# r9y9/gantts

Hardware: AMD Instinct MI355X
Metric: acoustic frames/sec per G+D GAN step (B=32,T=512) (higher is better)
Workload: dtype f32; 1 GPU; cfg2: TTS acoustic MLP G 425-512x3-187 + conditioned MLP D 483-256x3-1, Adagrad, MGE+ADV loss, global B=32 T=512 (32 sequences per GPU, strong scaling), fp32, dropout 0.5 (Philox); global_batch=32, per_gpu_batch=32, parallelism=dp1

## Files before the change

gantts_amd/_lib.py:

```python
import ctypes as C
import os

import torch

_HERE = os.path.dirname(os.path.abspath(__file__))
LIB_PATH = os.environ.get("GT_HIP_LIB") or os.path.join(_HERE, "libgantts_hip.so")

GT_OK, GT_ERR_INVALID, GT_ERR_HIP, GT_ERR_STATE, GT_ERR_DIM = 0, 1, 2, 3, 4
ROLE_G, ROLE_D = 0, 1
OPT_LSTM_PERSISTENT, OPT_LSTM_FWD_UNITS, OPT_LSTM_XCD_LOCAL, OPT_MATMUL_BF16, OPT_SPLIT_FIRST_LAYER = 2, 3, 4, 5, 6
OPT_COMM_D_ONE_MSG, OPT_COMM_EARLY_G, OPT_COMM_FORCE = 10, 11, 13
OPT_LAUNCH_RIDERS, OPT_COMM_CLOSE_INLINE, OPT_POLL_RESULTS = 14, 15, 16
OPT_COMM_TV_IN_SUMS, OPT_COMM_IPC, OPT_FUSED_DSTACK = 17, 18, 19
OPT_SRU_D_BF16 = 20
OPT_GAN_OBJECTIVE = 21
GAN_OBJECTIVES = {"bce": 0, "ls": 1, "hinge": 2, "wgan": 3}
GAN_OBJECTIVE_THRESHOLD = {"bce": 0.5, "ls": 0.5, "hinge": 0.0, "wgan": 0.0}
IPC_HANDLE_BYTES, IPC_MAX_WORLD = 64, 8
PROFILE_SLOTS = 16
LSTM_PATH_SLOTS, LSTM_PATH_STEPS, LSTM_PATH_DECLINED = 34, 32, 33
GEMM_PATH_SLOTS = 588
GEMM_B16_PATH_SLOTS = 66
SRU_PATH_SLOTS = 13
HEAD_PATH_SLOTS = 15
SN_MAX_LAYERS, SN_PATH_SLOTS = 17, 5
GP_MAX_LAYERS, GP_PATH_SLOTS = 16, 8
GRAD_PENALTIES = {None: 0, "r1": 1, "wgan-gp": 2}
(FRAME_MASK_SUM, FRAME_MASK_TOTAL, FRAME_SQERR, FRAME_G_LOSSES, FRAME_STATIC_GRAD, FRAME_FINALIZE_G, FRAME_FINALIZE_G_RIDER, FRAME_FINALIZE_D,
 FRAME_SCALE_INV_TV, FRAME_HIGHWAY_FWD, FRAME_HIGHWAY_BWD, FRAME_SIGMOID_GRAD, FRAME_DROPOUT_APPLY, FRAME_BUILD_ADV, FRAME_BUILD_CAT2, FRAME_REPITCH,
 FRAME_DENSE_COPY, FRAME_PAD_ROWS, FRAME_TRANSPOSE) = range(19)
FRAME_SCALARS = 26
CAST_PLAIN_F32, CAST_PLAIN_BF16, CAST_SEQDROP, CAST_CAT, CAST_CATDROP, CAST_MULTI = 0, 1, 2, 3, 4, 5
CAST_MAX_JOBS = 8
GEMM_ROUTE_FORWARD, GEMM_ROUTE_FORWARD_SEG, GEMM_ROUTE_BACKWARD_DATA, GEMM_ROUTE_WEIGHT_GRAD, GEMM_ROUTE_WEIGHT_GRAD_SPLIT = 0, 1, 2, 3, 4
ARCH_MLP, ARCH_IN2OUT, ARCH_LSTM, ARCH_SRU, ARCH_IN2OUT_RNN = 0, 1, 2, 3, 4
OPT_ADAGRAD, OPT_ADAM = 0, 1
OPT_SGD, OPT_RMSPROP, OPT_ADADELTA, OPT_ADAMW, OPT_ADAMAX = 2, 3, 4, 5, 6
OPT_NADAM, OPT_RADAM, OPT_RPROP, OPT_ASGD = 7, 8, 9, 10
OPTF_NESTEROV, OPTF_CENTERED, OPTF_AMSGRAD, OPTF_BUFFER_LIVE = 1, 2, 4, 8
OPTF_DECOUPLED_WD = 32
MLPG_VAR_PATH_SLOTS = 3
MAX_STREAMS = 8
MLPG_R_FROM_WINDOWS = 1
MLPG_MAX_WINDOW_SPAN = 32
COMM_ID_BYTES = 128
SCALE_NONE, SCALE_MINMAX, SCALE_MEANVAR = 0, 1, 2
ASSEMBLE_MAX_WINDOWS, ASSEMBLE_MAX_TAPS = 4, 9
CORPUS_STATS_SLAB, CORPUS_STATS_FANIN = 256, 64
LEDGER_SLOTS = 32
LEDGER_HAS_D, LEDGER_HAS_G, LEDGER_HAS_DIST = 1, 2, 4
LEDGER_ACOUSTIC, LEDGER_DURATION, LEDGER_VC = 0, 1, 2
LEDGER_KEYS = ("generator", "mse", "mge", "loss_real_d", "loss_fake_d", "loss_adv", "discriminator", "real_correct", "fake_correct",
               "mcd", "bap_mcd", "f0_rmse", "vuv_err", "dur_rmse", "d_updates", "g_updates")


class StreamConfig(C.Structure):
    _fields_ = [("n_streams", C.c_int32),
                ("stream_sizes", C.c_int32 * MAX_STREAMS),
                ("has_dynamic_features", C.c_int32 * MAX_STREAMS),
                ("num_windows", C.c_int32),
                ("adversarial_streams", C.c_int32 * MAX_STREAMS),
                ("mask_nth_mgc_for_adv_loss", C.c_int32),
                ("discriminator_linguistic_condition", C.c_int32),
                ("cond_dim", C.c_int32)]


class ModelDesc(C.Structure):
    _fields_ = [("arch", C.c_int32), ("in_dim", C.c_int32), ("out_dim", C.c_int32),
                ("num_hidden", C.c_int32), ("hidden_dim", C.c_int32), ("static_dim", C.c_int32),
                ("dropout", C.c_float), ("last_sigmoid", C.c_int32),
                ("bidirectional", C.c_int32), ("use_relu", C.c_int32),
                ("rnn_dropout", C.c_float), ("reserved_", C.c_int32),
                ("params", C.c_void_p), ("grads", C.c_void_p), ("n_params", C.c_int64)]


class OptimDesc(C.Structure):
    _fields_ = [("kind", C.c_int32), ("lr", C.c_float), ("weight_decay", C.c_float), ("eps", C.c_float),
                ("lr_decay", C.c_float), ("beta1", C.c_float), ("beta2", C.c_float),
                ("max_grad_norm", C.c_float), ("step", C.c_int64),
                ("state0", C.c_void_p), ("state1", C.c_void_p)]


class OptimDescEx(C.Structure):
    _fields_ = ([("kind", C.c_int32), ("flags", C.c_uint32)]
                + [(n, C.c_double) for n in ("lr", "weight_decay", "eps", "lr_decay", "beta1", "beta2", "momentum", "dampening", "alpha")]
                + [("max_grad_norm", C.c_float), ("reserved_", C.c_int32), ("step", C.c_int64),
                   ("state0", C.c_void_p), ("state1", C.c_void_p), ("state2", C.c_void_p)])


class OptimDescEx2(OptimDescEx):
    _fields_ = [(n, C.c_double) for n in ("momentum_decay", "etaminus", "etaplus", "step_size_min", "step_size_max", "lambd", "t0",
                                          "host_state0", "host_state1")]


class DResult(C.Structure):
    _fields_ = [("loss_d", C.c_float), ("loss_fake_d", C.c_float), ("loss_real_d", C.c_float),
                ("real_correct_count", C.c_float), ("fake_correct_count", C.c_float), ("grad_norm", C.c_float)]


class GResult(C.Structure):
    _fields_ = [("loss_mse", C.c_float), ("loss_mge", C.c_float), ("loss_adv", C.c_float),
                ("loss_g", C.c_float), ("grad_norm", C.c_float)]


class GemmCase(C.Structure):
    _fields_ = ([(n, C.c_int32) for n in ("route", "prec", "rows", "in_dim", "out_dim", "act", "drop")] + [("p", C.c_float)]
                + [("key0", C.c_uint32), ("key1", C.c_uint32)]
# ... 97 lines not shown

class GpCase(C.Structure):
    _fields_ = ([(n, C.c_int32) for n in ("kind", "L", "H", "cd", "Da", "ld_g")] + [("rows", C.c_int64), ("weight", C.c_float), ("inv_tv", C.c_float)]
                + [(n, C.c_void_p * GP_MAX_LAYERS) for n in ("W", "dW", "Hact", "a", "c")] + [("drop", DropSite * GP_MAX_LAYERS)]
                + [(n, C.c_void_p) for n in ("w_last", "dw_last", "mask", "g", "g_copy", "phi", "nrm", "sums", "rec")])


class CastJob(C.Structure):
    _fields_ = ([(n, C.c_void_p) for n in ("in_", "out", "outT")] + [("rows", C.c_int64), ("ldt", C.c_int64)]
                + [(n, C.c_int32) for n in ("ldi", "cols", "ldo", "pad_")])


class CastCase(C.Structure):
    _fields_ = ([(n, C.c_int32) for n in ("kind", "cols", "ldi", "ldo", "colsum_accumulate", "T", "cd", "ldf", "n_jobs", "pad_")]
                + [(n, C.c_int64) for n in ("rows", "ldt", "N", "row_off")]
                + [(n, C.c_void_p) for n in ("in_", "out", "outT", "colsum", "mul", "x", "fa", "fb", "idx")]
                + [("jobs", CastJob * CAST_MAX_JOBS)])


_P, _I, _F, _L = C.c_void_p, C.c_int, C.c_float, C.c_int64

class DistortionSums(C.Structure):
    _fields_ = [(n, C.c_double) for n in
                ("s_mcd", "s_bap", "s_f0", "n_voiced", "n_vuv_err", "s_mse", "n_frames")]


SIGNATURES = {
    "gt_last_error": (C.c_char_p, []),
    "gt_version": (C.c_char_p, []),
    "gt_engine_create": (_I, [C.POINTER(StreamConfig), C.POINTER(_P)]),
    "gt_engine_destroy": (None, [_P]),
    "gt_bind_model": (_I, [_P, _I, C.POINTER(ModelDesc)]),
    "gt_bind_optimizer": (_I, [_P, _I, C.POINTER(OptimDesc)]),
    "gt_bind_optimizer_ex": (_I, [_P, _I, C.POINTER(OptimDescEx)]),
    "gt_op_optim_step": (_I, [C.POINTER(OptimDescEx), _P, _P, _L, _P, C.POINTER(_F), _P]),
    "gt_set_training": (_I, [_P, _I, _I]),
    "gt_set_lr": (_I, [_P, _I, _F]),
    "gt_get_optimizer_step": (_I, [_P, _I, C.POINTER(_L)]),
    "gt_get_optimizer_scalars": (_I, [_P, _I, C.POINTER(C.c_double)]),
    "gt_op_optim_scalars": (_I, [C.POINTER(OptimDescEx), _L, C.POINTER(C.c_double)]),
    "gt_set_seed": (_I, [_P, C.c_uint64]),
    "gt_set_dropout_mask": (_I, [_P, _I, _I, _I, _P]),
    "gt_op_philox_mask": (_I, [_P, _I, _I, _I, _L, _F, _L, _I, _P, _P]),
    "gt_set_lengths": (_I, [_P, C.POINTER(_L), _I, _P]),
    "gt_invalidate_mlpg_cache": (_I, [_P]),
    "gt_set_mlpg_windows": (_I, [_P, _I, C.POINTER(C.c_int32), C.POINTER(C.c_int32), C.POINTER(C.c_double)]),
    "gt_zero_grad": (_I, [_P, _I]),
    "gt_apply_generator": (_I, [_P, _P, _P, _I, _I, _P, _P, _P]),
    "gt_update_discriminator": (_I, [_P, _P, _P, _P, _P, _I, _I, _I, _F, C.POINTER(DResult), _P]),
    "gt_update_generator": (_I, [_P, _P, _P, _P, _P, _P, _F, _P, _I, _I, _I, _F, _F, _F, C.POINTER(GResult), _P]),
    "gt_set_loss_normalizer": (_I, [_P, _F]),
    "gt_set_loss_normalizer_device": (_I, [_P, _P]),
    "gt_set_option": (_I, [_P, _I, _I]),
    "gt_set_weight_clip": (_I, [_P, _I, _F]),
    "gt_set_param_ema": (_I, [_P, _I, _P, _L, C.c_double]),
    "gt_set_param_ema_count": (_I, [_P, _I, _L]),
    "gt_get_param_ema_count": (_I, [_P, _I, C.POINTER(_L)]),
    "gt_op_optim_step_ema": (_I, [C.POINTER(OptimDescEx), _P, _P, _L, _P, C.POINTER(_F), _P, _L, C.c_double, _P]),
    "gt_set_spectral_norm": (_I, [_P, _I, _P, _P, _L, _L]),
    "gt_op_spectral_norm": (_I, [C.POINTER(SnCase), _P]),
    "gt_op_sn_project": (_I, [C.POINTER(SnCase), _P]),
    "gt_sn_path_counts": (_I, [C.POINTER(_L), _I]),
    "gt_set_grad_penalty": (_I, [_P, _I, _I, _F]),
    "gt_set_gp_epsilon": (_I, [_P, _P]),
    "gt_grad_penalty_result": (_I, [_P, C.POINTER(C.c_double), C.POINTER(C.c_double), C.POINTER(_L), _I]),
    "gt_grad_penalty_peek": (_I, [_P, _P, _P, _P]),
    "gt_op_grad_penalty": (_I, [C.POINTER(GpCase), _P]),
    "gt_gp_path_counts": (_I, [C.POINTER(_L), _I]),
    "gt_set_x_pitch": (_I, [_P, _I, _I]),
    "gt_set_tuning": (_I, [C.c_char_p, _I]),
    "gt_check_faults": (_I, [_P, _P]),
    "gt_lstm_path_counts": (_I, [_P, C.POINTER(_L), _I]),
    "gt_gemm_path_counts": (_I, [C.POINTER(_L), _I]),
    "gt_op_gemm_f32": (_I, [C.POINTER(GemmCase), _P]),
    "gt_gemm_b16_path_counts": (_I, [C.POINTER(_L), _I]),
    "gt_op_gemm_b16": (_I, [C.POINTER(GemmB16Case), _P]),
    "gt_op_cast_image": (_I, [C.POINTER(CastCase), _P]),
    "gt_sru_path_counts": (_I, [C.POINTER(_L), _I]),
    "gt_op_sru_scan": (_I, [C.POINTER(SruScanCase), _P]),
    "gt_op_sru_dx_adv_finish": (_I, [_P, _L, _I, _I, _P, _I, _P, _I, _P]),
    "gt_op_sru_input_mask": (_I, [_P, _I, _I, _F, C.c_uint32, C.c_uint32, _P, _I, _I, _P]),
    "gt_op_sru_input_dropout": (_I, [_P, _I, _P, _I, _I, _I, _I, _P, _P]),
    "gt_head_path_counts": (_I, [C.POINTER(_L), _I]),
    "gt_op_d_head": (_I, [C.POINTER(DHeadCase), _P]),
    "gt_op_dstack": (_I, [C.POINTER(DStackCase), _P]),
    "gt_op_frame": (_I, [C.POINTER(FrameCase), _P]),
    "gt_op_mlpg": (_I, [C.POINTER(MlpgCase), _P]),
    "gt_op_mlpg_band": (_I, [_P, _P, _I, C.POINTER(_F), _L, C.POINTER(C.c_int32), _P]),
    "gt_op_mlpg_var": (_I, [C.POINTER(MlpgVarCase), _P]),
    "gt_mlpg_var_path_counts": (_I, [C.POINTER(_L), _I]),
    "gt_op_assemble_batch": (_I, [C.POINTER(AssembleCase), _P]),
    "gt_op_assemble_shard": (_I, [C.POINTER(AssembleCase), C.POINTER(AssembleShard), _P]),
    "gt_corpus_stats_workspace_bytes": (_L, [_L, C.c_int32]),
    "gt_op_corpus_stats": (_I, [C.POINTER(CorpusStatsCase), _P]),
    "gt_clear_faults": (_I, [_P, _P]),
    "gt_comm_unique_id": (_I, [_P]),
    "gt_comm_init": (_I, [_P, _I, _I, _P]),
    "gt_comm_destroy": (_I, [_P]),
    "gt_comm_info": (_I, [_P, C.POINTER(_I), C.POINTER(_I)]),
    "gt_comm_trace": (_I, [_P, _I]),
    "gt_comm_trace_read": (_I, [_P, C.POINTER(C.c_double), _I, C.POINTER(_I)]),
    "gt_set_shard": (_I, [_P, _I, _I]),
    "gt_comm_ipc_export": (_I, [_P, _P]),
    "gt_comm_ipc_attach": (_I, [_P, _I, _I, _P]),
    "gt_comm_ipc_messages": (_I, [_P, C.POINTER(C.c_longlong)]),
    "gt_update_discriminator_begin": (_I, [_P, _P, _P, _P, _P, _I, _I, _I, _F, _P]),
    "gt_update_discriminator_end": (_I, [_P, _I, C.POINTER(DResult), _P]),
    "gt_update_generator_begin": (_I, [_P, _P, _P, _P, _P, _P, _F, _P, _I, _I, _I, _F, _F, _F, _P]),
    "gt_update_generator_end": (_I, [_P, _I, _F, _F, _F, C.POINTER(GResult), _P]),
    "gt_update_discriminator_result": (_I, [_P, C.POINTER(DResult)]),
    "gt_update_generator_result": (_I, [_P, C.POINTER(GResult)]),
    "gt_scalar_buffer": (_I, [_P, C.POINTER(_P), C.POINTER(_I)]),
    "gt_model_forward": (_I, [_P, _I, _P, _P, _I, _I, _P, _P, _P]),
    "gt_flush_generator_grads": (_I, [_P, _P]),
    "gt_op_sequence_mask": (_I, [_P, _I, _I, _P, _P]),
    "gt_op_masked_mse": (_I, [_P, _P, _P, _I, _I, _I, C.POINTER(_F), _P, _P]),
    "gt_compute_distortions": (_I, [_P, _P, _I, _P, _P, _I, C.POINTER(_I), C.POINTER(_I), _I, C.POINTER(_L), _I, _I,
                                    C.POINTER(DistortionSums), _P]),
    "gt_ledger_configure": (_I, [_P, _I, _I, C.POINTER(_I), C.POINTER(_I), _I, _P, _P, _I, C.c_double]),
    "gt_ledger_reset": (_I, [_P, _P]),
    "gt_ledger_add": (_I, [_P, _I, _P, _P, _P, _I, _I, _P]),
    "gt_ledger_read": (_I, [_P, C.POINTER(C.c_double), _P]),
    "gt_ledger_buffers": (_I, [_P, C.POINTER(_P), C.POINTER(_P)]),
    "gt_op_epoch_ledger": (_I, [_P, _P, _P, _I, _I, _I, C.c_double, _P]),
    "gt_host_wait_count": (_I, [_P, C.POINTER(C.c_longlong)]),
    "gt_op_gather_cols": (_I, [_P, _I, _P, _I, _P, _I, _I, _L, _P]),
    "gt_op_pad_sequences": (_I, [_P, _I, _P, _P, _I, _I, _P, _I, _P]),
    "gt_op_mlpg_forward": (_I, [_P, _P, _P, _I, _I, _P, _P]),
    "gt_op_mlpg_backward": (_I, [_P, _P, _P, _I, _I, _P, _P]),
    "gt_op_linear_forward": (_I, [_P, _I, _P, _P, _P, _I, _L, _I, _I, _I, _P, _F, _P]),
    "gt_op_linear_bf16": (_I, [_P, _P, _P, _L, _I, _I, _I, _P, _F, _P, _P, _P, _I, _P, _F, _P, _P, _P, _P, _P, _P]),
    "gt_profile_enable": (_I, [_I]),
    "gt_profile_read": (_I, [C.POINTER(C.c_double), C.POINTER(C.c_double), C.POINTER(_L)]),
    "gt_profile_bytes": (_I, [C.POINTER(C.c_double)]),
    "gt_op_linear_backward": (_I, [_P, _I, _P, _I, _P, _L, _I, _I, _P, _I, _P, _I, _P, _F, _P, _P, _P]),
}


def _build_if_missing():
    import fcntl
    import shutil
    import subprocess
    if os.path.isfile(LIB_PATH):
        return
    if shutil.which("hipcc") is None and not os.path.isfile("/opt/rocm/bin/hipcc"):
        return
    with open(os.path.join(_HERE, ".build.lock"), "w") as lock:
        fcntl.flock(lock, fcntl.LOCK_EX)
        try:
            if not os.path.isfile(LIB_PATH):
                subprocess.call(["make", "-j8", "-C", os.path.join(_HERE, "csrc")], stdout=subprocess.DEVNULL)
        finally:
            fcntl.flock(lock, fcntl.LOCK_UN)


def _load():
    _build_if_missing()
    if not os.path.isfile(LIB_PATH):
        raise ImportError(
            "gantts_amd: %s not found -- the HIP engine is the product and has no fallback. "
            "Build it: make -C %s" % (LIB_PATH, os.path.join(_HERE, "csrc")))
    lib = C.CDLL(LIB_PATH)
    for name, (res, args) in SIGNATURES.items():
        fn = getattr(lib, name)
        fn.restype, fn.argtypes = res, args
    return lib
# ... 30 lines not shown
```

gantts_amd/csrc/d_tail_args.hip.h:

```cpp
#pragma once
#include "dstack_f32.hip.h"

namespace gt {

struct HeadCall {
  int mode;
  long rows, n_real;
  const float* mask; long n_mask;
  float eps;
  bool want_grad;
  bool want_w;
  StepResults* early_res;
  int* defer_scalars;
  const double* tv_dev;
  unsigned ticket;
  bool unit_tv;
  int objective;
};

struct HeadSums {
  StepScalars* sc;
  HeadPartials* hp; long hp_cap;
  float* dw_partial; long dw_cap;
  float* dW; float* db;
  int accumulate;
  unsigned* ticket_dev;
};

struct HeadArgs {
  HeadCall c;
  HeadSums o;
  const void* H; int K;
  int ldh;
  int h_ld;
  bool has_act;
  DropoutSpec spec;
  const float* w; const float* bias;
  float* Dout;
  float* dH; int lddh;
  __bf16* dHb; int lddhb;
  __bf16* dHbT; long lddhbt;
};

struct DStackCall {
  HeadCall c;
  HeadSums o;
  int hidden_dim;
  DStackArgs a;
};

inline int d_head_blocks(long rows) { const long n = (rows + 31) / 32; return (int)(n < 1024 ? n : 1024); }

}
```

gantts_amd/csrc/eng_core.hip:

```cpp
#include "engine_internal.hip.h"

using namespace gt;
static thread_local char g_err[512] = "";
int fail(int code, const char* fmt, ...) {
  va_list ap;
  va_start(ap, fmt);
  vsnprintf(g_err, sizeof(g_err), fmt, ap);
  va_end(ap);
  return code;
}
extern "C" const char* gt_last_error(void) { return g_err; }
extern "C" const char* gt_version(void) { return "gantts_hip 0.1 (gfx950, f32 MFMA)"; }

int ensure_dyn_lds(const void* kernel, size_t bytes) {
  static std::mutex mu;
  static std::map<std::pair<const void*, int>, size_t> done;
  int dev = 0;
  HIPCHK(hipGetDevice(&dev));
  std::lock_guard<std::mutex> lk(mu);
  size_t& cur = done[std::make_pair(kernel, dev)];
  if (bytes > cur) {
    HIPCHK(hipFuncSetAttribute(kernel, hipFuncAttributeMaxDynamicSharedMemorySize, (int)bytes));
    cur = bytes;
  }
// ... 325 lines not shown
extern "C" int gt_set_training(gt_engine* e, int role, int training) {
  if (!e || role < 0 || role > 1) return fail(GT_ERR_INVALID, "bad argument");
  e->net[role].training = training != 0;
  return GT_OK;
}
extern "C" int gt_set_lr(gt_engine* e, int role, float lr) {
  if (!e || role < 0 || role > 1 || !e->net[role].has_opt) return fail(GT_ERR_INVALID, "no optimizer bound");
  e->net[role].od.lr = lr;
  return GT_OK;
}
extern "C" int gt_get_optimizer_step(gt_engine* e, int role, int64_t* step) {
  if (!e || role < 0 || role > 1 || !step) return fail(GT_ERR_INVALID, "bad argument");
  *step = e->net[role].step;
  return GT_OK;
}
extern "C" int gt_get_optimizer_scalars(gt_engine* e, int role, double out[2]) {
  if (!e || role < 0 || role > 1 || !out) return fail(GT_ERR_INVALID, "bad argument");
  Net& n = e->net[role];
  if (!n.has_opt) return fail(GT_ERR_INVALID, "no optimizer bound");
  optim_host_scalars(n.od, n.step, &n.hs_cache, out);
  return GT_OK;
}
extern "C" int gt_set_seed(gt_engine* e, uint64_t seed) {
  if (!e) return fail(GT_ERR_INVALID, "null engine");
  e->seed = seed;
  e->step_counter = 0;
  e->dx_pitched.forget(); e->gx_pitched.forget(); e->cx_dense.forget();
  return GT_OK;
}
extern "C" int gt_set_dropout_mask(gt_engine* e, int role, int pass, int layer, const float* mask) {
  if (!e || role < 0 || role > 1 || pass < 0 || pass > (role == GT_ROLE_D ? 3 : 2) || layer < 0 || layer > 15) return fail(GT_ERR_INVALID, "bad argument");
  e->net[role].inj[pass][layer] = mask;
  return GT_OK;
}
extern "C" int gt_set_option(gt_engine* e, int option, int value) {
  if (!e) return fail(GT_ERR_INVALID, "null engine");
  switch (option) {
    case GT_OPT_LSTM_PERSISTENT: e->lstm_persistent = value != 0; return GT_OK;
    case GT_OPT_LSTM_FWD_UNITS: e->lstm_fwd_upc = value; return GT_OK;
    case GT_OPT_LSTM_XCD_LOCAL: e->lstm_xcd_local = value != 0; return GT_OK;
    case GT_OPT_SPLIT_FIRST_LAYER:
      if (e->opt_split_first != (value != 0)) invalidate_d_images(e);
      e->opt_split_first = value != 0;
      return GT_OK;
    case GT_OPT_COMM_D_ONE_MSG: e->opt_comm_d_one_msg = value != 0; return GT_OK;
    case GT_OPT_COMM_EARLY_G: e->opt_comm_early_g = value != 0; return GT_OK;
    case GT_OPT_COMM_FORCE: e->opt_comm_force = value != 0; return GT_OK;
    case GT_OPT_COMM_CLOSE_INLINE: e->opt_comm_close_inline = value != 0; return GT_OK;
    case GT_OPT_COMM_IPC: e->opt_comm_ipc = value != 0; return GT_OK;
    case GT_OPT_FUSED_DSTACK: e->opt_fused_dstack = value < 0 ? 0 : value > 2 ? 2 : value; return GT_OK;
    case GT_OPT_COMM_TV_IN_SUMS: e->opt_comm_tv_in_sums = value != 0; return GT_OK;
    case GT_OPT_POLL_RESULTS: e->opt_poll_results = value != 0; return GT_OK;
    case GT_OPT_LAUNCH_RIDERS: e->opt_launch_riders = value != 0; return GT_OK;
    case GT_OPT_MATMUL_BF16:
      if (e->matmul_bf16 != (value != 0)) {
        invalidate_d_images(e);
        e->g_pass_valid = false; e->leak.drop(); e->cx_dense.forget(); e->results.forget_begin();
      }
      e->matmul_bf16 = value != 0;
      return GT_OK;
    case GT_OPT_SRU_D_BF16:
      if (value != 0 && value != 1) return fail(GT_ERR_INVALID, "GT_OPT_SRU_D_BF16 takes 0 or 1, not %d", value);
      if (e->sru_d_bf16 != (value != 0)) { invalidate_d_images(e); e->leak.drop(); e->results.forget_begin(); }
      e->sru_d_bf16 = value != 0;
      return GT_OK;
    case GT_OPT_GAN_OBJECTIVE:
      if (value < 0 || value >= GAN_OBJ_COUNT) return fail(GT_ERR_INVALID, "GT_OPT_GAN_OBJECTIVE takes 0 (bce), 1 (ls), 2 (hinge) or 3 (wgan), not %d", value);
      if (e->net[GT_ROLE_D].bound) CHK(gan_objective_fits(value, e->net[GT_ROLE_D].d.last_sigmoid != 0));
      if (e->gan_objective != value) { e->leak.drop(); e->results.forget_begin(); }
      e->gan_objective = value;
      return GT_OK;
  }
  return fail(GT_ERR_INVALID, "unknown option %d", option);
}
GtTuning& gt_tuning() {
  static GtTuning t = [] {
    GtTuning v;
    auto geti = [](const char* n, int d) { const char* s = getenv(n); return s && s[0] ? atoi(s) : d; };
    v.gemm_pair = geti("GT_GEMM_PAIR", v.gemm_pair); v.pair_order = geti("GT_PAIR_ORDER", v.pair_order);
    { const char* s = getenv("GT_GEMM_TILES"); v.gemm_tiles_big = s && !strcmp(s, "big") ? 1 : 0; }
    v.gemm_unaligned = geti("GT_GEMM_UNALIGNED", v.gemm_unaligned); v.tn_wgs = geti("GT_TN_WGS", v.tn_wgs); v.tn_split_wgs = geti("GT_TN_SPLIT_WGS", v.tn_split_wgs); v.split_fused = geti("GT_SPLIT_FUSED", v.split_fused);
    v.b16_tiles = geti("GT_B16_TILES", v.b16_tiles); v.b16_wg_tile = geti("GT_B16_WG_TILE", v.b16_wg_tile); v.b16_dma = geti("GT_B16_DMA", v.b16_dma);
    v.mlpg_fpl = geti("GT_MLPG_FPL", v.mlpg_fpl); v.mlpg_tt = geti("GT_MLPG_TT", v.mlpg_tt); v.sru_coop = geti("GT_SRU_COOP", v.sru_coop); v.sru_cs_waves = geti("GT_SRU_CS_WAVES", v.sru_cs_waves); v.leak_rider = geti("GT_LEAK_RIDER", v.leak_rider);
    v.head_vec = geti("GT_HEAD_VEC", v.head_vec);
    v.lstm_bt = geti("GT_LSTM_BT", v.lstm_bt);
    if (v.lstm_bt != 8 && v.lstm_bt != 16) v.lstm_bt = 0;
    return v;
  }();
  return t;
}
extern "C" int gt_set_tuning(const char* name, int value) {
  if (!name) return fail(GT_ERR_INVALID, "null name");
  GtTuning& t = gt_tuning();
  struct { const char* n; int* p; } tab[] = {
      {"gemm_pair", &t.gemm_pair}, {"pair_order", &t.pair_order}, {"gemm_tiles_big", &t.gemm_tiles_big}, {"gemm_unaligned", &t.gemm_unaligned},
      {"tn_wgs", &t.tn_wgs}, {"tn_split_wgs", &t.tn_split_wgs}, {"split_fused", &t.split_fused}, {"b16_tiles", &t.b16_tiles},
      {"b16_wg_tile", &t.b16_wg_tile}, {"b16_dma", &t.b16_dma}, {"mlpg_fpl", &t.mlpg_fpl}, {"mlpg_tt", &t.mlpg_tt}, {"sru_coop", &t.sru_coop}, {"sru_cs_waves", &t.sru_cs_waves}, {"leak_rider", &t.leak_rider}, {"head_vec", &t.head_vec}};
  if (!strcmp(name, "lstm_bt")) {
    if (value != 0 && value != 8 && value != 16) return fail(GT_ERR_INVALID, "lstm_bt must be 0 (by shape), 8 or 16, not %d", value);
    t.lstm_bt = value;
    return GT_OK;
  }
  if (!strcmp(name, "sru_lw")) { t.sru_coop = value >= 2; return GT_OK; }
  for (auto& e : tab) if (!strcmp(e.n, name)) { *e.p = value; return GT_OK; }
  return fail(GT_ERR_INVALID, "unknown tuning knob '%s'", name);
}
extern "C" int gt_set_x_pitch(gt_engine* e, int ld_generator_input, int ld_condition) {
  if (!e || ld_generator_input < 0 || ld_condition < 0) return fail(GT_ERR_INVALID, "bad argument");
  e->ld_gx = ld_generator_input; e->ld_cx = ld_condition;
  return GT_OK;
}
extern "C" int gt_set_loss_normalizer(gt_engine* e, float tv) {
  if (!e) return fail(GT_ERR_INVALID, "null engine");
  e->norm.set_override(tv);
  return GT_OK;
}
extern "C" int gt_set_loss_normalizer_device(gt_engine* e, const double* tv_dev) {
  if (!e) return fail(GT_ERR_INVALID, "null engine");
  e->norm.set_total_dev(tv_dev);
  return GT_OK;
}
extern "C" int gt_set_lengths(gt_engine* e, const int64_t* lengths_host, int B, void* stream) {
  if (!e || !lengths_host || B < 1) return fail(GT_ERR_INVALID, "bad argument");
  hipStream_t s = (hipStream_t)stream;
  e->h_lengths.resize(B);
  for (int b = 0; b < B; ++b) {
    if (lengths_host[b] < 0 || lengths_host[b] > 0x3fffffff) return fail(GT_ERR_INVALID, "length out of range");
    e->h_lengths[b] = (int)lengths_host[b];
  }
  if (2 * B > e->len_cap) {
    HIPCHK(hipStreamSynchronize(s));
    const int cap = std::max(64, 2 * B + B);
    for (int i = 0; i < gt_engine::LEN_RING; ++i) {
      if (e->len_ev[i]) HIPCHK(hipEventSynchronize(e->len_ev[i]));
      if (e->len_host[i]) { HIPCHK(hipHostFree(e->len_host[i])); e->len_host[i] = nullptr; }
      HIPCHK(hipHostMalloc((void**)&e->len_host[i], (size_t)cap * sizeof(int)));
      if (!e->len_ev[i]) HIPCHK(hipEventCreateWithFlags(&e->len_ev[i], hipEventDisableTiming));
    }
    e->len_cap = cap;
  }
  const int slot = (e->len_slot + 1) % gt_engine::LEN_RING;
  HIPCHK(hipEventSynchronize(e->len_ev[slot]));
  memcpy(e->len_host[slot], e->h_lengths.data(), (size_t)B * sizeof(int));
  memcpy(e->len_host[slot] + B, e->h_lengths.data(), (size_t)B * sizeof(int));
  CHK(e->len_dev[slot].ensure((size_t)e->len_cap * sizeof(int)));
  HIPCHK(hipMemcpyAsync(e->len_dev[slot].p, e->len_host[slot], (size_t)2 * B * sizeof(int), hipMemcpyHostToDevice, s));
  HIPCHK(hipEventRecord(e->len_ev[slot], s));
  e->len_slot = slot;
  return GT_OK;
}

extern "C" int gt_zero_grad(gt_engine* e, int role) {
  if (!e || role < 0 || role > 1) return fail(GT_ERR_INVALID, "bad argument");
  e->net[role].grads_dirty = false;
  e->ws[role].sdefer.reset(false);
  e->norm.forget();
  if (role == GT_ROLE_G) e->leak.drop();
  return GT_OK;
}
extern "C" int gt_scalar_buffer(gt_engine* e, double** dev_ptr, int* n) {
  if (!e || !dev_ptr || !n) return fail(GT_ERR_INVALID, "bad argument");
  *dev_ptr = &e->sc()->s_real;
  *n = 7;
  return GT_OK;
}

DropoutSpec philox_site_spec(gt_engine* e, int role, int pass, int layer, uint64_t step, float p, long half_rows) {
  DropoutSpec d = no_drop();
  d.p = p;
  d.scale = 1.f / (1.f - p);
  d.mode = DROP_PHILOX;
  const double th = (double)p * 65536.0 + 0.5;
  d.thresh = th >= 65535.0 ? 65535u : (uint32_t)th;
  const uint64_t site = step * 64ULL + (uint64_t)(role * 32 + pass * 16 + layer);
  uint32_t rk = 0;
  if (e->dp_world > 1) {
    const int T = e->chk_T, B = e->chk_B;
    const long groups = ((long)B * T / 16) * e->dp_world * 2;
    if (T > 0 && T % 16 == 0 && groups < (1L << 21) && (half_rows == 0 || half_rows == (long)B * T)) {
      d.dp_t16 = (uint32_t)(T / 16);
// ... 90 lines not shown
```

gantts_amd/csrc/eng_gemm_f32.hip:

```cpp
#include "engine_internal.hip.h"
#include <atomic>

using namespace gt;
int launch_gemm_nt(const GemmArgs& g, int bm, int bn, int prec, hipStream_t s);
int launch_gemm_nn(const GemmArgs& g, int bm, int bn, int prec, hipStream_t s);
int launch_gemm_tn(const GemmArgs& g, int bm, int bn, int nslab, int prec, hipStream_t s);
int launch_gemm_pair(const GemmArgs& nn_in, const GemmArgs& tn_in, int nslab, int prec, hipStream_t s);
int launch_gemm_tn_pair(const GemmArgs& g1_in, const GemmArgs& g2_in, int nslab1, int nslab2, int prec, hipStream_t s, const GemmArgs* rider, bool* rode);
int gemm_cu_count() {
  static std::map<int, int> cus;
  int dev = 0;
  if (hipGetDevice(&dev) != hipSuccess) return 256;
  auto it = cus.find(dev);
  if (it != cus.end()) return it->second;
  hipDeviceProp_t prop;
  const int n = hipGetDeviceProperties(&prop, dev) == hipSuccess ? prop.multiProcessorCount : 256;
  cus[dev] = n;
  return n;
}

static std::atomic<int64_t> g_gemm_paths[GT_GEMM_PATH_SLOTS];
void gemm_path_count(int slot) { g_gemm_paths[slot].fetch_add(1, std::memory_order_relaxed); }
extern "C" int gt_gemm_path_counts(int64_t* counts, int reset) {
  for (int i = 0; i < GT_GEMM_PATH_SLOTS; ++i) {
    const int64_t v = reset ? g_gemm_paths[i].exchange(0, std::memory_order_relaxed) : g_gemm_paths[i].load(std::memory_order_relaxed);
    if (counts) counts[i] = v;
  }
  return GT_OK;
}

static int pick_bn(int N) { return (cdiv(N, 64) * 64 < cdiv(N, 128) * 128) ? 64 : 128; }

static int gemm_tile_mode() { return gt_tuning().gemm_tiles_big; }
static bool gemm_unaligned_ok() { return gt_tuning().gemm_unaligned != 0; }
bool gemm_vec_ok(const float* p, int ld, bool k_contiguous) {
  if (k_contiguous && gemm_unaligned_ok()) return true;
  return (ld % 4 == 0) && (((uintptr_t)p) % 16 == 0);
}
bool gemm_wide_store_ok(int kind, const GemmArgs& g) {
  if (kind == GEMM_TN) return false;
  if (gemm_unaligned_ok()) return true;
  return (g.ldc % 4 == 0) && (((uintptr_t)g.C) % 16 == 0) &&
         (kind != GEMM_NN || g.act == ACT_NONE || ((g.ldh % 4 == 0) && (((uintptr_t)g.H) % 16 == 0)));
}
bool gemm_small_tiles_ok() { return gemm_tile_mode() == 0; }


int launch_gemm(int kind, const GemmArgs& g, int prec, hipStream_t s) {
  if (g.M <= 0 || g.N <= 0 || g.K <= 0) return fail(GT_ERR_INVALID, "empty GEMM");
  if (kind != GEMM_NT && kind != GEMM_NN) return fail(GT_ERR_INVALID, "launch_gemm: forward and backward-data products only");
  const bool nt = kind == GEMM_NT;
  const bool vec = gemm_vec_ok(g.A, g.lda, true) && gemm_vec_ok(g.B, g.ldb, nt);
  if (vec && g.M > 64 && gemm_small_tiles_ok()) return nt ? launch_gemm_nt(g, 64, 64, prec, s) : launch_gemm_nn(g, 64, 64, prec, s);
  const int bn = pick_bn(g.N);
  int bm = 128;
  if (g.M > 64) {
    const long t128 = (long)cdiv(g.M, 128) * cdiv(g.N, bn), t64 = (long)cdiv(g.M, 64) * cdiv(g.N, bn);
    const double c128 = (double)cdiv(t128, 512), c64 = 0.55 * (double)cdiv(t64, bn == 64 ? 1024 : 768);
    if (c64 < c128) bm = 64;
  }
  return nt ? launch_gemm_nt(g, bm, bn, prec, s) : launch_gemm_nn(g, bm, bn, prec, s);
}
static int launch_gemm_slabs(const GemmArgs& g, int tile_m, int nslab, int prec, hipStream_t s) {
  if (g.M <= 0 || g.N <= 0 || g.K <= 0) return fail(GT_ERR_INVALID, "empty GEMM");
  return tile_m == 64 ? launch_gemm_tn(g, 64, 64, nslab, prec, s) : launch_gemm_tn(g, 128, pick_bn(g.N), nslab, prec, s);
}

DropoutSpec no_drop() {
  DropoutSpec d;
  memset(&d, 0, sizeof(d));
  d.mode = DROP_NONE;
  d.scale = 1.f;
  return d;
}
static GemmArgs gemm_args(const float* A, int lda, const float* B, int ldb, float* C, int ldc, long M, int N, int K) {
  GemmArgs g;
  memset(&g, 0, sizeof(g));
  g.A = A; g.lda = lda; g.B = B; g.ldb = ldb; g.C = C; g.ldc = ldc; g.M = (int)M; g.N = N; g.K = K;
  g.drop = no_drop();
  return g;
}
int plain_product(int kind, const float* A, int lda, const float* B, int ldb, float* C, int ldc, long M, int N, int K, bool accumulate, int prec,
                  hipStream_t s) {
  GemmArgs g = gemm_args(A, lda, B, ldb, C, ldc, M, N, K);
  g.accumulate = accumulate ? 1 : 0;
  return launch_gemm(kind, g, prec, s);
}

int linear_forward(const float* X, int ldx, const float* W, int ldw, const float* b, float* Y, int ldy, long rows, int in, int out, int act,
                   const DropoutSpec& drop, int prec, hipStream_t s, const float* addm, int ld_addm, long addm_wrap, bool accumulate) {
  GemmArgs g = gemm_args(X, ldx, W, ldw, Y, ldy, rows, out, in);
  g.bias = b; g.act = act; g.drop = drop; g.accumulate = accumulate ? 1 : 0;
  if (addm) { g.addm = addm; g.ld_addm = ld_addm; g.addm_wrap = (int)addm_wrap; }
  return launch_gemm(GEMM_NT, g, prec, s);
}
int linear_forward_seg(const float* x, int ldx, long wrap, int cd, const float* adv, int ld_adv, long rows, const float* W, int ldw, int in,
                       const float* b, float* Y, int ldy, int out, int act, const DropoutSpec& drop, int prec, hipStream_t s) {
  GemmArgs g = gemm_args(x, ldx, W, ldw, Y, ldy, wrap, out, cd);
  g.bias = b; g.act = act; g.drop = drop;
  g.A_seg = adv; g.lda_seg = ld_adv; g.B_seg = W + cd; g.K_seg = in - cd;
  g.dual_rows = rows == 2 * wrap ? (int)wrap : 0;
  return launch_gemm(GEMM_NT, g, prec, s);
}
GemmArgs backward_data_args(const float* dZ, int lddz, const float* W, int ldw, int col0, float* dX, int lddx,
                                   long rows, int out, int ncols, int act_prev, const float* H, int ldh, const DropoutSpec& drop) {
  GemmArgs g = gemm_args(dZ, lddz, W + col0, ldw, dX, lddx, rows, ncols, out);
  g.act = act_prev; g.H = H; g.ldh = ldh; g.drop = drop;
  return g;
}
int linear_backward_data(const float* dZ, int lddz, const float* W, int ldw, int col0, float* dX, int lddx,
                                long rows, int out, int ncols, int act_prev, const float* H, int ldh,
                                const DropoutSpec& drop, int prec, hipStream_t s) {
  return launch_gemm(GEMM_NN, backward_data_args(dZ, lddz, W, ldw, col0, dX, lddx, rows, out, ncols, act_prev, H, ldh, drop), prec, s);
}
static bool gemm_pair_enabled() { return gt_tuning().gemm_pair != 0; }
static bool gemm_pair_ok(const GemmArgs& nn) {
  return gemm_pair_enabled() && gemm_small_tiles_ok() && nn.M > 64 && gemm_vec_ok(nn.A, nn.lda, true) && gemm_vec_ok(nn.B, nn.ldb);
}


int slab_defer_flush(SlabDefer& d, hipStream_t s) {
  if (d.jobs.n > 0) {
    gemm_path_count(GEMM_PATH_REDUCE_MULTI);
    hipLaunchKernelGGL(slab_reduce_multi_kernel, dim3(d.blocks), dim3(256), 0, s, d.jobs);
    LAUNCH_CHECK();
  }
  d.jobs.n = 0; d.blocks = 0; d.used = 0;
  return GT_OK;
}
int slab_place(SlabDefer* defer, Scratch& slabs, int nslab, int out, int in, const float* dW, bool accumulate, hipStream_t s, SlabSet* set) {
  const long stride = (long)out * in;
  const size_t need = (((size_t)nslab * stride + (size_t)nslab * out) * sizeof(float) + 255) & ~(size_t)255;
  const bool can4 = stride % 4 == 0 && ((uintptr_t)dW) % 16 == 0;
  float* base = nullptr;
  if (defer && defer->active && accumulate) { CHK(slab_defer_flush(*defer, s)); defer = nullptr; }
  if (defer && defer->active && can4) {
    if (defer->jobs.n == SLAB_MAX_JOBS || defer->used + need > defer->pool.bytes) {
      CHK(slab_defer_flush(*defer, s));
      if (need > defer->pool.bytes) CHK(defer->pool.ensure(std::max(need * 4, (size_t)64 << 20)));
    }
    base = (float*)((char*)defer->pool.p + defer->used);
    defer->used += need;
  } else {
    defer = nullptr;
    CHK(slabs.ensure(need));
    base = slabs.as<float>();
  }
  *set = SlabSet{base, base + (size_t)nslab * stride, stride, need, nslab, out, can4, defer};
  return GT_OK;
}
int slab_combine(const SlabSet& t, float* dW, float* db, bool accumulate, hipStream_t s) {
  const int acc = accumulate ? 1 : 0;
  if (t.can4) {
    const int main_blocks = cdiv(t.stride / 4, 256), bias_blocks = db ? cdiv(t.out, 256) : 0;
    if (SlabDefer* d = t.defer) {
      SlabJob& J = d->jobs.j[d->jobs.n++];
      J.slabs = t.base; J.slab_stride = t.stride; J.n4 = t.stride / 4; J.out = dW; J.bslabs = t.bias; J.bout = db;
      J.nslab = t.nslab; J.accumulate = acc; J.nb = t.out; J.main_blocks = main_blocks; J.block0 = d->blocks; J.pad_ = 0;
      d->blocks += main_blocks + bias_blocks;
      return GT_OK;
    }
    gemm_path_count(GEMM_PATH_REDUCE4);
    hipLaunchKernelGGL(slab_reduce4_kernel, dim3(main_blocks + bias_blocks), dim3(256), 0, s, t.base, t.stride, t.nslab, t.stride / 4, dW, acc,
                       (const float*)t.bias, t.out, db, main_blocks);
    LAUNCH_CHECK();
    return GT_OK;
  }
  gemm_path_count(GEMM_PATH_REDUCE);
  hipLaunchKernelGGL(slab_reduce_kernel, dim3(cdiv(t.stride, 256)), dim3(256), 0, s, t.base, t.stride, t.nslab, t.stride, dW, acc);
  LAUNCH_CHECK();
  if (db) {
    gemm_path_count(GEMM_PATH_REDUCE_SMALL);
    hipLaunchKernelGGL(slab_reduce_small_kernel, dim3(cdiv(t.out, 64)), dim3(1024), 0, s, t.bias, (long)t.out, t.nslab, t.out, db, acc);
    LAUNCH_CHECK();
  }
  return GT_OK;
}
int linear_backward_weight(const float* dZ, int lddz, const float* X, int ldx, long rows, int out, int in,
                                  float* dW, float* db, bool accumulate, Scratch& slabs, Scratch& colp, int prec, hipStream_t s,
                                  SlabDefer* defer, const GemmArgs* ride_along, bool* rode) {
  if (rode) *rode = false;
  if (dW) {
    const bool t64 = gemm_vec_ok(dZ, lddz) && gemm_vec_ok(X, ldx) && gemm_small_tiles_ok();
    const int bn = t64 ? 64 : pick_bn(in);
    const int tiles = cdiv(out, t64 ? 64 : 128) * cdiv(in, bn);
    const int slab_wgs = gt_tuning().tn_wgs;
    int nslab = std::max(1, slab_wgs / tiles);
    const int max_slab = (int)((rows + 255) / 256);
    if (nslab > max_slab) nslab = max_slab;
    if (nslab < 1) nslab = 1;
    int k_chunk = cdiv(cdiv(rows, nslab), GEMM_BK) * GEMM_BK;
    nslab = cdiv(rows, k_chunk);
    SlabSet set;
    CHK(slab_place(defer, slabs, nslab, out, in, dW, accumulate, s, &set));
    GemmArgs g = gemm_args(dZ, lddz, X, ldx, set.base, in, out, in, (int)rows);
    g.k_chunk = k_chunk; g.slab_stride = set.stride;
    g.colsum_slab = db ? set.bias : nullptr;
    if (t64 && ride_along && rode && gemm_pair_ok(*ride_along)) {
      CHK(launch_gemm_pair(*ride_along, g, nslab, prec, s));
      *rode = true;
    } else {
      CHK(launch_gemm_slabs(g, t64 ? 64 : 128, nslab, prec, s));
    }
    return slab_combine(set, dW, db, accumulate, s);
  }
  if (db) {
    const int rows_per_blk = 128;
    const int nblk = cdiv(rows, rows_per_blk);
    CHK(colp.ensure((size_t)nblk * out * sizeof(float)));
    gemm_path_count(GEMM_PATH_COLSUM_PARTIAL);
    hipLaunchKernelGGL(colsum_partial_kernel, dim3(nblk, cdiv(out, 64)), dim3(256), 0, s, dZ, lddz, rows, out, rows_per_blk,
                       colp.as<float>());
    LAUNCH_CHECK();
    gemm_path_count(GEMM_PATH_COLSUM_FINALIZE);
    hipLaunchKernelGGL(colsum_finalize_kernel, dim3(cdiv(out, 256)), dim3(256), 0, s, colp.as<float>(), nblk, out, db,
                       accumulate ? 1 : 0);
    LAUNCH_CHECK();
  }
  return GT_OK;
}


int linear_backward_weight_split(const float* dZ, int lddz, long rows, long wrap, const float* xp, int ldxp, int cd,
                                 const float* adv, int ld_adv, int Da, int out, float* dW, float* db, bool accumulate,
                                 Scratch& slabs, int prec, hipStream_t s, SlabDefer* defer, const GemmArgs* rider, bool* rode) {
  if (rode) *rode = false;
  if (rows != wrap && rows != 2 * wrap) return fail(GT_ERR_INVALID, "split weight gradient: rows must be one or two halves");
  if (!gemm_vec_ok(dZ, lddz) || !gemm_vec_ok(xp, ldxp) || !gemm_vec_ok(adv, ld_adv) || prec != PREC_F32)
    return fail(GT_ERR_INVALID, "split weight gradient: operands must be 16-byte loadable (float32 products)");
  const int in = cd + Da;
  const int tiles = cdiv(out, 64) * (cdiv(cd, 64) + cdiv(Da, 64));
  int nslab = std::max(1, gt_tuning().tn_split_wgs / tiles);
  nslab = std::min<long>(nslab, std::max<long>(1, wrap / 256));
  const int kc1 = cdiv(cdiv(wrap, nslab), GEMM_BK) * GEMM_BK;
  const int ns1 = cdiv(wrap, kc1);
  const int kc2 = cdiv(cdiv(rows, ns1), GEMM_BK) * GEMM_BK;
  const int ns2 = cdiv(rows, kc2);
  SlabSet set;
  CHK(slab_place(defer, slabs, ns1, out, in, dW, accumulate, s, &set));
  if (ns2 < ns1)
    HIPCHK(hipMemsetAsync(set.base, 0, set.bytes, s));
  GemmArgs g1 = gemm_args(dZ, lddz, xp, ldxp, set.base, in, out, cd, (int)wrap);
  g1.A2 = rows == 2 * wrap ? dZ + wrap * (long)lddz : nullptr;
  g1.k_chunk = kc1; g1.slab_stride = set.stride;
  GemmArgs g2 = g1;
  g2.A2 = nullptr; g2.B = adv; g2.ldb = ld_adv; g2.C = set.base + cd; g2.N = Da; g2.K = (int)rows; g2.k_chunk = kc2;
  g2.colsum_slab = db ? set.bias : nullptr;
  if (g1.A2) {
    CHK(launch_gemm_tn_pair(g1, g2, ns1, ns2, prec, s, rider, rode));
  } else {
    CHK(launch_gemm_slabs(g1, 64, ns1, prec, s));
    CHK(launch_gemm_slabs(g2, 64, ns2, prec, s));
  }
  return slab_combine(set, dW, db, accumulate, s);
}
```

gantts_amd/csrc/eng_gemm_f32_pair.hip:

```cpp
#include "gemm_f32_launch.hip.h"

int launch_gemm_pair(const GemmArgs& nn_in, const GemmArgs& tn_in, int nslab, int prec, hipStream_t s) {
  GemmArgs nn = nn_in, tn = tn_in;
  nn.wide_store = gemm_wide_store_ok(GEMM_NN, nn) ? 1 : 0;
  tn.wide_store = 0;
  nn.n_tiles_m = cdiv(nn.M, 64); nn.n_tiles_n = cdiv(nn.N, 64);
  tn.n_tiles_m = cdiv(tn.M, 64); tn.n_tiles_n = cdiv(tn.N, 64);
  const int n1 = nn.n_tiles_m * nn.n_tiles_n, n2 = tn.n_tiles_m * tn.n_tiles_n * nslab;
  const bool bf16 = prec == PREC_BF16;
  const size_t lds = bf16 ? std::max(gemm_lds_bytes<GEMM_NN, 64, 64, PREC_BF16>(), gemm_lds_bytes<GEMM_TN, 64, 64, PREC_BF16>())
                          : std::max(gemm_lds_bytes<GEMM_NN, 64, 64>(), gemm_lds_bytes<GEMM_TN, 64, 64>());
  const int am = bf16 ? GEMM_A_RUNTIME : (nn.act == ACT_NONE ? GEMM_A_NONE : ((nn.act == ACT_LEAKY_DROPOUT && nn.drop.mode == DROP_PHILOX) ? GEMM_A_LEAKY_PHILOX : GEMM_A_RUNTIME));
  const void* kern = bf16 ? (const void*)gemm_pair_kernel<PREC_BF16> : (am == GEMM_A_NONE ? (const void*)gemm_pair_kernel<PREC_F32, GEMM_A_NONE> :
                     (am == GEMM_A_LEAKY_PHILOX ? (const void*)gemm_pair_kernel<PREC_F32, GEMM_A_LEAKY_PHILOX> : (const void*)gemm_pair_kernel<PREC_F32>));
  CHK(ensure_dyn_lds(kern, lds));
  GemmProfiler::Rec rec;
  if (g_prof.wants(5)) {
    rec.kind = 5; rec.bn = 64; rec.am = -1; rec.flops = 2.0 * nn.M * nn.N * nn.K + 2.0 * tn.M * tn.N * tn.K;
    rec.bytes = gemm_algorithmic_bytes(GEMM_NN, nn) + gemm_algorithmic_bytes(GEMM_TN, tn);
    rec.e0 = g_prof.get(); rec.e1 = g_prof.get();
    HIPCHK(hipEventRecord(rec.e0, s));
  }
  const int tn_first = gt_tuning().pair_order;
  const int grid = n1 + n2;
  gemm_path_count(GEMM_PATH_PAIR + (bf16 ? 3 : am == GEMM_A_NONE ? 0 : am == GEMM_A_LEAKY_PHILOX ? 1 : 2));
  if (bf16) hipLaunchKernelGGL(gemm_pair_kernel<PREC_BF16>, dim3(grid), dim3(GEMM_THREADS), lds, s, nn, tn, n1, tn_first);
  else if (am == GEMM_A_NONE) hipLaunchKernelGGL((gemm_pair_kernel<PREC_F32, GEMM_A_NONE>), dim3(grid), dim3(GEMM_THREADS), lds, s, nn, tn, n1, tn_first);
  else if (am == GEMM_A_LEAKY_PHILOX) hipLaunchKernelGGL((gemm_pair_kernel<PREC_F32, GEMM_A_LEAKY_PHILOX>), dim3(grid), dim3(GEMM_THREADS), lds, s, nn, tn, n1, tn_first);
  else      hipLaunchKernelGGL(gemm_pair_kernel<PREC_F32>, dim3(grid), dim3(GEMM_THREADS), lds, s, nn, tn, n1, tn_first);
  LAUNCH_CHECK();
  if (g_prof.wants(5)) { HIPCHK(hipEventRecord(rec.e1, s)); g_prof.recs.push_back(rec); }
  return GT_OK;
}

int launch_gemm_tn_pair(const GemmArgs& g1_in, const GemmArgs& g2_in, int nslab1, int nslab2, int prec, hipStream_t s, const GemmArgs* rider, bool* rode) {
  GemmArgs g1 = g1_in, g2 = g2_in, g3;
  memset(&g3, 0, sizeof(g3));
  int n3 = 0;
  if (rode) *rode = false;
  if (rider && rider->act == ACT_NONE && !rider->accumulate && rider->M > 0 && gemm_vec_ok(rider->A, rider->lda, true) && prec == PREC_F32 &&
      gemm_small_tiles_ok()) {
    g3 = *rider;
    g3.wide_store = gemm_wide_store_ok(GEMM_NN, g3) ? 1 : 0;
    g3.n_tiles_m = cdiv(g3.M, 64); g3.n_tiles_n = cdiv(g3.N, 64);
    n3 = g3.n_tiles_m * g3.n_tiles_n;
    if (rode) *rode = true;
  }
  g1.wide_store = g2.wide_store = 0;
  g1.n_tiles_m = cdiv(g1.M, 64); g1.n_tiles_n = cdiv(g1.N, 64);
  g2.n_tiles_m = cdiv(g2.M, 64); g2.n_tiles_n = cdiv(g2.N, 64);
  const int n1 = g1.n_tiles_m * g1.n_tiles_n * nslab1, n2 = g2.n_tiles_m * g2.n_tiles_n * nslab2;
  const size_t lds = std::max(gemm_lds_bytes<GEMM_TN, 64, 64>(), gemm_lds_bytes<GEMM_NN, 64, 64>());
  CHK(ensure_dyn_lds((const void*)gemm_tn_pair_kernel<PREC_F32>, lds));
  GemmProfiler::Rec rec;
  if (g_prof.wants(6)) {
    rec.kind = 6; rec.bn = 64; rec.am = -1; rec.flops = 2.0 * g1.M * g1.N * g1.K + 2.0 * g2.M * g2.N * g2.K + (n3 ? 2.0 * g3.M * g3.N * g3.K : 0.0);
    rec.bytes = gemm_algorithmic_bytes(GEMM_TN, g1) + 4.0 * (double)g1.M * g1.K + gemm_algorithmic_bytes(GEMM_TN, g2) + (n3 ? gemm_algorithmic_bytes(GEMM_NN, g3) : 0.0);
    rec.e0 = g_prof.get(); rec.e1 = g_prof.get();
    HIPCHK(hipEventRecord(rec.e0, s));
  }
  gemm_path_count(GEMM_PATH_TN_PAIR + (n3 > 0 ? 1 : 0));
  hipLaunchKernelGGL(gemm_tn_pair_kernel<PREC_F32>, dim3(n1 + n2 + n3), dim3(GEMM_THREADS), lds, s, g1, g2, n1, g3, n3);
  LAUNCH_CHECK();
  if (g_prof.wants(6)) { HIPCHK(hipEventRecord(rec.e1, s)); g_prof.recs.push_back(rec); }
  return GT_OK;
}
```

gantts_amd/csrc/eng_step.hip:

```cpp
#include "engine_internal.hip.h"
#include "d_tail_args.hip.h"
#include "d_tail_launch.hip.h"
#include <atomic>

using namespace gt;
static int stage_injected(gt_engine* e, int role, int layer, const int* passes, int npass, long rows_each, int width,
                          const float** out, hipStream_t s) {
  Net& n = e->net[role];
  *out = nullptr;
  if (!n.training || n.d.dropout <= 0.f) return GT_OK;
  bool any = false, all = true;
  for (int i = 0; i < npass; ++i) { any |= n.inj[passes[i]][layer] != nullptr; all &= n.inj[passes[i]][layer] != nullptr; }
  if (!any) return GT_OK;
  if (!all) return fail(GT_ERR_INVALID, "injected dropout masks must be given for every pass of a step or for none");
  if (npass == 1) { *out = n.inj[passes[0]][layer]; return GT_OK; }
  const size_t per_layer = (size_t)npass * rows_each * width * sizeof(float);
  CHK(e->dmask.ensure(per_layer * n.d.num_hidden));
  float* base = (float*)((char*)e->dmask.p + per_layer * layer);
  for (int i = 0; i < npass; ++i)
    HIPCHK(hipMemcpyAsync(base + (size_t)i * rows_each * width, n.inj[passes[i]][layer], (size_t)rows_each * width * sizeof(float),
                          hipMemcpyDeviceToDevice, s));
  *out = base;
  return GT_OK;
}

struct FirstSplit {
  const float* x; int ldx; int cd;
  const float* xp; int ldxp;
  const float* adv; int ld_adv;
  long wrap;
};
static int step_copy(gt_engine* e, StepCopy& M, const float* p, int ld, int cols, long rows, int ldo, bool dense, const float** out, hipStream_t s) {
  if (!M.holds(p, ld, cols, rows, e->step_counter)) {
    CHK(M.buf.ensure((size_t)rows * ldo * sizeof(float)));
    if (dense) launch_copy_cols(p, ld, 0, M.buf.as<float>(), ldo, 0, rows, cols, s);
    else launch_repitch(p, ld, cols, rows, M.buf.as<float>(), ldo, s);
    LAUNCH_CHECK();
    M.built(p, ld, cols, rows, e->step_counter);
  }
  *out = M.buf.as<float>();
  return GT_OK;
}
static int pitched_rows(gt_engine* e, StepCopy& M, const float* p, int ld, int cols, long rows, const float** out, int* ldo, hipStream_t s) {
  if (gemm_vec_ok(p, ld)) { *out = p; *ldo = ld; return GT_OK; }
  *ldo = (cols + 3) & ~3;
  return step_copy(e, M, p, ld, cols, rows, *ldo, false, out, s);
}

static int stack_forward(gt_engine* e, int role, const float* in, int ld_in, long rows, const int* passes, int npass, long rows_each, std::vector<DropoutSpec>& specs, hipStream_t s,
                         const FirstSplit* fs = nullptr, int max_layers = 1 << 30 ) {
  Net& n = e->net[role];
  std::vector<Scratch>& acts = e->ws[role].act;
  const int prec = product_prec(e, role);
  specs.resize(n.hidden.size());
  const float* cur = in;
  int ld = ld_in;
  for (size_t l = 0; l < n.hidden.size(); ++l) {
    const Lin& L = n.hidden[l];
    CHK(acts[l].ensure((size_t)rows * L.out * sizeof(float)));
    const float* inj = nullptr;
    CHK(stage_injected(e, role, (int)l, passes, npass, rows_each, L.out, &inj, s));
    specs[l] = drop_spec(e, role, passes[0], (int)l, inj, L.out, npass == 2 ? rows_each : 0);
    if ((int)l >= max_layers) continue;
    if (l == 0 && fs && specs[l].mode == DROP_PHILOX && gt_tuning().split_fused && gemm_vec_ok(fs->x, fs->ldx, true) &&
        gemm_vec_ok(L.W, L.in, true) && gemm_vec_ok(fs->adv, fs->ld_adv, true) && fs->wrap > 64 && gemm_small_tiles_ok() &&
        prec == PREC_F32 && (rows == fs->wrap || rows == 2 * fs->wrap)) {
      CHK(linear_forward_seg(fs->x, fs->ldx, fs->wrap, fs->cd, fs->adv, fs->ld_adv, rows, L.W, L.in, L.in, L.b, acts[l].as<float>(), L.out, L.out,
                             ACT_LEAKY_DROPOUT, specs[l], prec, s));
      cur = acts[l].as<float>();
      ld = L.out;
      continue;
    }
    if (l == 0 && fs) {
      const int Da = L.in - fs->cd;
      CHK(e->d_pre.ensure((size_t)fs->wrap * L.out * sizeof(float)));
      CHK(linear_forward(fs->x, fs->ldx, L.W, L.in, L.b, e->d_pre.as<float>(), L.out, fs->wrap, fs->cd, L.out, ACT_NONE, no_drop(), prec, s));
      CHK(linear_forward(fs->adv, fs->ld_adv, L.W + fs->cd, L.in, nullptr, acts[l].as<float>(), L.out, rows, Da, L.out, ACT_LEAKY_DROPOUT, specs[l],
                         prec, s, e->d_pre.as<float>(), L.out, fs->wrap));
      cur = acts[l].as<float>();
      ld = L.out;
      continue;
    }
    const float* W = L.W;
    int ldw = L.in;
    if (l == 0 && (L.in & 3) && gemm_vec_ok(cur, ld) && !gemm_vec_ok(L.W, L.in, true) && prec == PREC_F32) {
      ldw = (L.in + 3) & ~3;
      CHK(e->ws[role].w0pad.ensure((size_t)L.out * ldw * sizeof(float)));
      launch_pad_rows(L.W, L.in, L.out, e->ws[role].w0pad.as<float>(), ldw, s);
      LAUNCH_CHECK();
      W = e->ws[role].w0pad.as<float>();
    }
    CHK(linear_forward(cur, ld, W, ldw, L.b, acts[l].as<float>(), L.out, rows, L.in, L.out, ACT_LEAKY_DROPOUT, specs[l], prec, s));
    cur = acts[l].as<float>();
    ld = L.out;
  }
  return GT_OK;
}


static int stack_backward(gt_engine* e, int role, const float* in, int ld_in, long rows, const std::vector<DropoutSpec>& specs, float* cur, float* other, bool want_w,
                          float* dX, int lddx, int col0, int ncols, long row0, long nrows, hipStream_t s, const FirstSplit* fs = nullptr) {
  Net& n = e->net[role];
  std::vector<Scratch>& acts = e->ws[role].act;
  const int L = (int)n.hidden.size(), prec = product_prec(e, role);
  for (int l = L - 1; l >= 0; --l) {
    const Lin& Lr = n.hidden[l];
    const float* Xin = l > 0 ? acts[l - 1].as<float>() : in;
    const int ldx = l > 0 ? n.hidden[l - 1].out : ld_in;
    bool rode = false;
    GemmArgs nn;
    if (l > 0) nn = backward_data_args(cur, Lr.out, Lr.W, Lr.in, 0, other, Lr.in, rows, Lr.out, Lr.in, ACT_LEAKY_DROPOUT,
                                       acts[l - 1].as<float>(), Lr.in, specs[l - 1]);
    if (want_w && l == 0 && fs) {
      GemmArgs leak;
      if (dX) leak = backward_data_args(cur + row0 * Lr.out, Lr.out, Lr.W, Lr.in, col0, dX, lddx, nrows, Lr.out, ncols, ACT_NONE, nullptr, 0, no_drop());
      CHK(linear_backward_weight_split(cur, Lr.out, rows, fs->wrap, fs->xp, fs->ldxp, fs->cd, fs->adv, fs->ld_adv, Lr.in - fs->cd, Lr.out,
                                       Lr.dW, Lr.db, n.grads_dirty, e->slabs, prec, s, &e->ws[role].sdefer, dX && gt_tuning().leak_rider ? &leak : nullptr, &rode));
      CHK(comm_grads_ready(e, role, Lr.dW, (long)Lr.out * Lr.in + Lr.out, s));
    } else if (want_w) {
      CHK(linear_backward_weight(cur, Lr.out, Xin, ldx, rows, Lr.out, Lr.in, Lr.dW, Lr.db, n.grads_dirty, e->slabs, e->colp, prec, s, &e->ws[role].sdefer,
                                 l > 0 ? &nn : nullptr, &rode));
      CHK(comm_grads_ready(e, role, Lr.dW, (long)Lr.out * Lr.in + Lr.out, s));
      if (l == 1 && (role == GT_ROLE_G || !e->opt_comm_d_one_msg)) CHK(comm_flush(e, role, s));
    }
    if (l > 0) {
      if (!rode) CHK(launch_gemm(GEMM_NN, nn, prec, s));
      std::swap(cur, other);
    } else if (dX && !rode) {
      CHK(linear_backward_data(cur + row0 * Lr.out, Lr.out, Lr.W, Lr.in, col0, dX, lddx, nrows, Lr.out, ncols, ACT_NONE, nullptr, 0,
                               no_drop(), prec, s));
    }
  }
  return GT_OK;
}

static bool use_b16(const gt_engine* e, int role) {
  const Net& n = e->net[role];
  if (!e->matmul_bf16 || !n.bound || n.d.arch != GT_ARCH_MLP || (n.d.hidden_dim & 7)) return false;
  return true;
}
static int refresh_shadows(gt_engine* e, int role, bool with_last, hipStream_t s) {
  Net& n = e->net[role];
  auto& sh = e->ws[role].wsh;
  sh.resize(n.hidden.size() + 1);
  CastJobs jobs;
  jobs.n = 0; jobs.pad_ = 0;
  int blocks = 0;
  auto flush = [&]() -> int {
    CHK(cast_transpose_multi(jobs, blocks, s));
    jobs.n = 0; blocks = 0;
    return GT_OK;
  };
  for (size_t l = 0; l <= n.hidden.size(); ++l) {
    if (l == n.hidden.size() && !with_last) break;
    const Lin& L = l < n.hidden.size() ? n.hidden[l] : n.last;
    LinShadow& w = sh[l];
    CHK(w.ensure(L.out, L.in));
    if (jobs.n == CAST_MAX_JOBS) CHK(flush());
    CHK(cast_jobs_add(jobs, blocks, L.W, L.in, L.out, L.in, w.r(), w.ldw, w.t(), w.ldwt));
  }
  return flush();
}
static int stack_forward_b16(gt_engine* e, int role, const __bf16* in_b, int ld_in, long rows, const int* passes, int npass, long rows_each,
                             std::vector<DropoutSpec>& specs, bool want_t, hipStream_t s) {
  Net& n = e->net[role];
  std::vector<B16Img>& acts = e->ws[role].actb;
  const std::vector<LinShadow>& wsh = e->ws[role].wsh;
  specs.resize(n.hidden.size());
  acts.resize(n.hidden.size());
  const __bf16* cur = in_b;
  int ld = ld_in;
  for (size_t l = 0; l < n.hidden.size(); ++l) {
    const Lin& L = n.hidden[l];
    CHK(acts[l].ensure(rows, L.out, want_t));
    const float* inj = nullptr;
    CHK(stage_injected(e, role, (int)l, passes, npass, rows_each, L.out, &inj, s));
    specs[l] = drop_spec(e, role, passes[0], (int)l, inj, L.out, npass == 2 ? rows_each : 0);
    CHK(b16_forward(cur, ld, rows, wsh[l].r(), wsh[l].ldw, L.out, L.in, L.b, ACT_LEAKY_DROPOUT, specs[l], B16Dst(acts[l], want_t), s));
    cur = acts[l].r();
    ld = acts[l].ld;
  }
  return GT_OK;
}
static int stack_backward_b16(gt_engine* e, int role, const __bf16* in_t, long ld_int, long rows, const std::vector<DropoutSpec>& specs, int cur, bool want_w,
                              float* dX, int lddx, int col0, int ncols, long row0, long nrows, hipStream_t s) {
  Net& n = e->net[role];
  std::vector<B16Img>& acts = e->ws[role].actb;
  const std::vector<LinShadow>& wsh = e->ws[role].wsh;
  for (int l = (int)n.hidden.size() - 1; l >= 0; --l) {
    const Lin& Lr = n.hidden[l];
    B16Img& dz = e->dz_b[cur];
    if (want_w) {
      const __bf16* XT = l > 0 ? acts[l - 1].t() : in_t;
      const long ldxt = l > 0 ? acts[l - 1].ldt : ld_int;
      CHK(weight_grad_b16(dz.t(), dz.ldt, XT, ldxt, rows, Lr.out, Lr.in, Lr.dW, Lr.db, n.grads_dirty, e->slabs, s, &e->ws[role].sdefer));
      CHK(comm_grads_ready(e, role, Lr.dW, (long)Lr.out * Lr.in + Lr.out, s));
      if (l == 1 && (role == GT_ROLE_G || !e->opt_comm_d_one_msg)) CHK(comm_flush(e, role, s));
    }
    if (l > 0) {
      B16Img& nx = e->dz_b[cur ^ 1];
      CHK(nx.ensure(rows, Lr.in, want_w));
      CHK(b16_backward_data(dz.r(), dz.ld, rows, wsh[l].t(), wsh[l].ldwt, Lr.in, Lr.out, ACT_LEAKY_DROPOUT, &acts[l - 1], specs[l - 1],
                            B16Dst(nx, want_w), s));
      cur ^= 1;
// ... 104 lines not shown
    }
    CHK(out_layer_forward(e, GT_ROLE_G, mlp_top(e, GT_ROLE_G, b16), N, y_hat, s));
  }
  if (is_i2o(G.d.arch)) {
    if (!R) return fail(GT_ERR_INVALID, "In2OutHighwayNet needs the MLPG matrix R (models.py:54)");
    const int sd = G.d.static_dim;
    const MlpgBand* band;
    CHK(ensure_band(e, R, T, s, &band));
    if (stash) e->g_band = band;
    CHK(e->tx.ensure((size_t)N * sd * sizeof(float)));
    CHK(e->gx.ensure((size_t)N * sd * sizeof(float)));
    CHK(linear_forward(x, G.d.in_dim, G.gate.W, sd, G.gate.b, e->tx.as<float>(), sd, N, sd, sd, ACT_SIGMOID, no_drop(), product_prec(e, GT_ROLE_G), s));
    CHK(mlpg_forward(e, gsrc, G.d.out_dim, e->d_scol_i2o, e->d_sstride_i2o, sd, e->gx.as<float>(), sd, B, T, *band, s));
    launch_highway_forward(x, G.d.in_dim, e->tx.as<float>(), sd, e->gx.as<float>(), sd, y_hat_static, sd, N, sd, s);
    LAUNCH_CHECK();
  } else {
    if (G.d.out_dim != e->Dout_cfg)
      return fail(GT_ERR_DIM, "You probably have specified wrong dimention params.");
    if (R) {
      const MlpgBand* band;
      CHK(ensure_band(e, R, T, s, &band));
      if (stash) e->g_band = band;
      CHK(mlpg_forward(e, y_hat, G.d.out_dim, e->d_scol, e->d_sstride, e->Ds, y_hat_static, e->Ds, B, T, *band, s));
    } else {
      if (e->Ds != G.d.out_dim) return fail(GT_ERR_INVALID, "R is None but the stream config has dynamic features");
      if (stash) e->g_band = nullptr;
      launch_copy_cols(y_hat, G.d.out_dim, 0, y_hat_static, G.d.out_dim, 0, N, G.d.out_dim, s);
      LAUNCH_CHECK();
    }
  }
  return GT_OK;
}

extern "C" int gt_apply_generator(gt_engine* e, const float* x, const float* R, int B, int T, float* y_hat,
                                  float* y_hat_static, void* stream) {
  CHK(check_common(e, B, T));
  Net& G = e->net[GT_ROLE_G];
  if (!G.bound) return fail(GT_ERR_STATE, "generator not bound");
  if (!x || !y_hat || !y_hat_static) return fail(GT_ERR_INVALID, "null tensor");
  hipStream_t s = (hipStream_t)stream;
  CHK(fault_seen(e));
  e->step_counter++;
  e->B = B; e->T = T; e->N = (long)B * T;
  e->g_pass_valid = false;
  invalidate_d_images(e);
  e->dx_pitched.forget(); e->gx_pitched.forget(); e->cx_dense.forget();
  e->norm.forget();
  CHK(generator_forward(e, x, R, B, T, y_hat, y_hat_static, true, s, e->ws[GT_ROLE_G].specs));
  e->last_x = e->gx_dense_on ? e->gx_dense.as<float>() : x;
  e->last_yhat = y_hat; e->last_yhs = y_hat_static;
  e->g_pass_valid = true;
  return GT_OK;
}

int cond_dim(gt_engine* e) {
  if (!e->cfg.discriminator_linguistic_condition) return 0;
  if (e->cfg.cond_dim > 0) return e->cfg.cond_dim;
  return e->net[GT_ROLE_D].bound ? e->net[GT_ROLE_D].d.in_dim - e->Da : 0;
}
static int d_in_dim(gt_engine* e) { return e->Da + cond_dim(e); }

static int build_cat(gt_engine* e, const float* x, const float* feats, int ld_feats, long row0, long N, int ldc, hipStream_t s) {
  float* dst = e->dcat.as<float>() + row0 * ldc;
  const int cd = cond_dim(e);
  if (cd > 0) {
    launch_copy_cols(x, cd, 0, dst, ldc, 0, N, cd, s);
    LAUNCH_CHECK();
  }
  hipLaunchKernelGGL(gather_cols_kernel, dim3(cdiv(N * e->Da, 256)), dim3(256), 0, s, feats, ld_feats, 0, e->d_adv_cols, dst, ldc,
                     cd, (int)N, e->Da);
  LAUNCH_CHECK();
  return GT_OK;
}

static std::atomic<int64_t> g_head_paths[GT_HEAD_PATH_SLOTS];
void head_path_count(int slot) { g_head_paths[slot].fetch_add(1, std::memory_order_relaxed); }
extern "C" int gt_head_path_counts(int64_t* counts, int reset) {
  for (int i = 0; i < GT_HEAD_PATH_SLOTS; ++i) {
    const int64_t v = reset ? g_head_paths[i].exchange(0, std::memory_order_relaxed) : g_head_paths[i].load(std::memory_order_relaxed);
    if (counts) counts[i] = v;
  }
  return GT_OK;
}

int launch_head_finalize(const HeadCall& c, const HeadSums& o, int nblk, int K, hipStream_t s) {
  const bool w = c.want_grad && c.want_w;
  if (c.defer_scalars && !w) { *c.defer_scalars = nblk; return GT_OK; }
  if (nblk > o.hp_cap || (w && (long)nblk * K > o.dw_cap)) return fail(GT_ERR_INVALID, "discriminator head: partial buffers too small for %d workgroups", nblk);
  const int cgw = (w && nblk >= 512) ? 16 : 64;
  const int n_dw = cdiv(K, cgw), extra = cgw == 16 ? 1 : 0;
  hipLaunchKernelGGL(d_head_finalize_kernel, dim3(n_dw + extra), dim3(1024), 0, s, o.hp, o.dw_partial, nblk, K, c.mode, o.sc,
                     w ? o.dW : (float*)nullptr, w ? o.db : (float*)nullptr, o.accumulate, c.early_res,
                     c.ticket ? o.ticket_dev : (unsigned*)nullptr, c.ticket, cgw, extra ? n_dw : 0);
  LAUNCH_CHECK();
  head_path_count(cgw == 16 ? HEAD_PATH_FINALIZE16 : HEAD_PATH_FINALIZE64);
  return GT_OK;
}

int launch_dstack_pass(const DStackCall& k, hipStream_t s) {
  const HeadCall& c = k.c;
  const int H = k.hidden_dim;
  const bool d_step = c.mode == HEAD_D_STEP;
  const int nblk = dstack_panels(c.rows);
  if (nblk > k.o.hp_cap || (d_step && c.want_grad && (long)nblk * H > k.o.dw_cap))
    return fail(GT_ERR_INVALID, "fused discriminator stack: partial buffers too small for %d panels", nblk);
  DStackArgs a = k.a;
  a.mode = d_step ? DSTACK_D_STEP : DSTACK_G_ADV; a.rows = (int)c.rows; a.n_real = (int)c.n_real;
  for (int l = 0; l < a.L && l < DS_MAXL; ++l)
    if (a.drop[l].mode == DROP_BUFFER && a.drop[l].ld_mask != H) return fail(GT_ERR_INVALID, "injected dropout mask pitch");
  a.mask = c.mask; a.n_mask = (int)c.n_mask; a.eps = c.eps; a.unit_tv = c.unit_tv ? 1 : 0; a.tv_dev = c.tv_dev;
  a.sc = k.o.sc; a.want_grad = c.want_grad ? 1 : 0; a.hp = k.o.hp;
  a.dw_partial = (d_step && c.want_grad) ? k.o.dw_partial : (float*)nullptr;
  if (!d_step && c.want_grad && !a.gadv) return fail(GT_ERR_INVALID, "fused discriminator stack: no gradient buffer");
  CHK(launch_dstack(a, H, s, c.objective));
  return launch_head_finalize(c, k.o, nblk, H, s);
}

int launch_d_head(const HeadArgs& a, hipStream_t s) {
  const int nblk = d_head_blocks(a.c.rows);
  if (nblk > a.o.hp_cap || (long)nblk * a.K > a.o.dw_cap) return fail(GT_ERR_INVALID, "discriminator head: partial buffers too small for %d workgroups", nblk);
  if (a.c.objective == GAN_OBJ_BCE) CHK(head_launch_by_k<GAN_OBJ_BCE>(a, nblk, s));
  else CHK(launch_d_head_objective(a, nblk, s));
  return launch_head_finalize(a.c, a.o, nblk, a.K, s);
}

static int head_sums(gt_engine* e, int nblk, int K, bool dw, HeadSums* o) {
  Net& D = e->net[GT_ROLE_D];
  CHK(e->headp.ensure((size_t)nblk * sizeof(HeadPartials)));
  if (dw) CHK(e->headw.ensure((size_t)nblk * K * sizeof(float)));
  o->sc = e->sc();
  o->hp = e->headp.as<HeadPartials>(); o->hp_cap = (long)(e->headp.bytes / sizeof(HeadPartials));
  o->dw_partial = e->headw.as<float>(); o->dw_cap = (long)(e->headw.bytes / sizeof(float));
  o->dW = D.last.dW; o->db = D.last.db; o->accumulate = D.grads_dirty ? 1 : 0;
  o->ticket_dev = e->results.ticket_dev();
  return GT_OK;
}

static bool d_fused_ok(gt_engine* e, long rows) {
  Net& D = e->net[GT_ROLE_D];
  if (e->opt_fused_dstack < 2 && dstack_panels(rows) < gemm_cu_count()) return false;
  if (!e->opt_fused_dstack || D.d.arch != GT_ARCH_MLP || product_prec(e, GT_ROLE_D) != PREC_F32 || !dstack_hidden_ok(D.d.hidden_dim)) return false;
  if (D.hidden.empty() || (int)D.hidden.size() > DS_MAXL || D.last.out != 1 || e->Da < 1 || e->Da > 64) return false;
  for (size_t l = 0; l < D.hidden.size(); ++l)
    if (D.hidden[l].out != D.d.hidden_dim || (l > 0 && D.hidden[l].in != D.d.hidden_dim)) return false;
  return true;
}
static int run_dstack(gt_engine* e, const HeadCall& c, float* gadv, hipStream_t s) {
  Net& D = e->net[GT_ROLE_D];
  NetWs& W = e->ws[GT_ROLE_D];
  const int H = D.d.hidden_dim, L = (int)D.hidden.size();
  const bool d_step = c.mode == HEAD_D_STEP;
  DStackCall k;
  memset(&k, 0, sizeof(k));
  k.c = c; k.hidden_dim = H;
  CHK(head_sums(e, dstack_panels(c.rows), H, d_step && c.want_grad, &k.o));
  CHK(e->dout.ensure((size_t)c.rows * sizeof(float)));
  DStackArgs& a = k.a;
  a.L = L;
  a.H0 = W.act[0].as<float>();
  for (int l = 0; l < L; ++l) { a.W[l] = D.hidden[l].W; a.b[l] = D.hidden[l].b; a.drop[l] = W.specs[l]; }
  a.w_last = D.last.W; a.b_last = D.last.b; a.Dout = e->dout.as<float>();
  if (d_step) {
    for (int l = 1; l + 1 < L; ++l) a.Hout[l] = W.act[l].as<float>();
    a.dZtop = e->dzA.as<float>();
    if (e->gp.kind == GP_R1 && c.want_grad && L > 1) a.Hout[L - 1] = W.act[L - 1].as<float>();
  } else {
    a.W0 = D.hidden[0].W; a.ldw0 = D.hidden[0].in; a.col0 = cond_dim(e); a.Da = e->Da; a.gadv = gadv; a.ld_gadv = e->Da;
  }
  return launch_dstack_pass(k, s);
}

struct HeadAct {
  const void* H; int K;
  int h_ld;
  bool has_act;
  DropoutSpec spec;
  float* dH;
  B16Img* dz_img; bool dz_t;
// ... 141 lines not shown
  bool fused;
  bool sru_d16;
  bool needs_f32_image;
  bool want_w;
  int passes[2], npass;
  long N, rows;
  int B, nseq, T, K0, ldc, H;
  const float* x;
  const float* real; const float* fake; int ldf;
  FirstSplit fs;
  CatSrc cat0;
  const float* img;
  const float* top; int ld_top;
};
static int d_pass_plan(gt_engine* e, const float* x, const float* real, const float* fake, int ldf, int npass, int B, int T, bool want_w, DPass* out) {
  Net& D = e->net[GT_ROLE_D];
  if (D.d.in_dim != d_in_dim(e))
    return fail(GT_ERR_DIM, "discriminator in_dim %d != adversarial input width %d (train.py:760-768)", D.d.in_dim, d_in_dim(e));
  const int cd = cond_dim(e);
  if (e->cfg.discriminator_linguistic_condition) {
    if (!x) return fail(GT_ERR_INVALID, "discriminator_linguistic_condition is set but x is null");
    if (cd <= 0) return fail(GT_ERR_DIM, "discriminator in_dim too small for linguistic conditioning");
  }
  DPass& p = *out;
  memset(&p, 0, sizeof(p));
  p.kind = D.d.arch == GT_ARCH_SRU ? D_SRU : has_lstm_body(D.d.arch) ? D_LSTM : use_b16(e, GT_ROLE_D) ? D_MLP_B16 : D_MLP_F32;
  p.npass = npass; p.passes[0] = npass == 2 ? 0 : 2; p.passes[1] = 1;
  p.B = B; p.T = T; p.N = (long)B * T; p.rows = npass * p.N; p.nseq = npass * B;
  p.K0 = D.d.in_dim; p.ldc = (p.K0 + 3) & ~3; p.H = D.d.hidden_dim;
  p.want_w = want_w; p.x = x; p.real = real; p.fake = fake; p.ldf = ldf;
  p.split = p.kind == D_MLP_F32 && d_split_ok(e, x);
  p.fused = p.kind == D_MLP_F32 && d_fused_ok(e, p.rows);
  p.sru_d16 = p.kind == D_SRU && sru_b16(e, GT_ROLE_D);
  p.needs_f32_image = p.kind == D_LSTM || (p.kind == D_SRU && sru_d_needs_f32_input(e)) || (p.kind == D_MLP_F32 && !p.split);
  if (p.split) { p.fs.x = x; p.fs.ldx = cx_pitch(e); p.fs.cd = cd; p.fs.ld_adv = (e->Da + 3) & ~3; p.fs.wrap = p.N; }
  CatSrc& c = p.cat0;
  c.x = x; c.cd = cd; c.fa = npass == 2 ? real : fake; c.fb = fake; c.ldf = ldf; c.idx = e->d_adv_cols; c.N = p.N; c.row_off = npass == 2 ? 0 : p.N;
  return GT_OK;
}

struct TvPlan {
  enum Route { KNOWN, LOCAL, ALLREDUCE, IN_SUMS } route;
  bool ride, head_reads;
  const float* mask; long N;
  TvPlan(gt_engine* e, const DPass& p, const float* mask_, bool steps) : mask(mask_), N(p.N) {
    const bool comm = comm_on(e), fused = e->results.early && e->opt_launch_riders;
    route = e->norm.known(mask, N) ? KNOWN : !comm || e->norm.given() ? LOCAL : fused && e->opt_comm_tv_in_sums && steps ? IN_SUMS : ALLREDUCE;
    ride = p.split && (route == IN_SUMS || (route == ALLREDUCE && fused) || (route == LOCAL && fused && !comm));
    head_reads = e->opt_launch_riders;
  }
  int before_input(gt_engine* e, hipStream_t s) const {
    if (ride || route == KNOWN || route == LOCAL) return GT_OK;
    if (route == ALLREDUCE) return e->norm.start(e, mask, N, s);
    launch_mask_total(mask, N, &e->sc()->tv_sum, s);
    LAUNCH_CHECK();
    return GT_OK;
  }
  void ride_on(gt_engine* e, BuildAdvArgs& ba) const {
    ba.tv_mask = ride ? mask : (const float*)nullptr; ba.tv_n = N; ba.tv_override = e->norm.override(); ba.sc = e->sc();
    ba.tv_total = !ride || route == LOCAL ? (double*)nullptr : route == IN_SUMS ? &e->sc()->tv_sum : e->norm.reduced();
  }
  int rode(gt_engine* e, hipStream_t s) const {
    if (ride && route == LOCAL) e->norm.note(mask, N);
    return ride && route == ALLREDUCE ? e->norm.send(e, s) : GT_OK;
  }
  int before_head(gt_engine* e, HeadCall& hc, hipStream_t s) const {
    LossNormaliser& n = e->norm;
    hc.unit_tv = route == IN_SUMS;
    switch (route) {
      case KNOWN: return GT_OK;
      case LOCAL: return n.ensure(e, mask, N, s);
      case ALLREDUCE:
        CHK(n.join(e, s));
        if (!head_reads) return n.file(e, mask, N, n.reduced(), s);
        hc.tv_dev = n.reduced();
        break;
      case IN_SUMS: break;
    }
    n.note(mask, N);
    return GT_OK;
  }
  double* early_sums(StepScalars* sc) const { return route == IN_SUMS ? &sc->tv_sum : &sc->s_real; }      int n_early_sums() const { return route == IN_SUMS ? 5 : 4; }
};
static int d_pass_input(gt_engine* e, DPass& p, const TvPlan* tv , hipStream_t s) {
  const long N = p.N;
  const bool both = p.npass == 2;
  const long row0 = both ? 0 : N;
  if (!p.split) {
    CHK(dense_cx(e, &p.x, N, s));
    p.cat0.x = p.x;
  }
  if (both) invalidate_d_images(e);
  if (p.kind == D_MLP_B16) {
    CHK(e->dcat_b.ensure(2 * N, p.K0, p.want_w));
    if (both || !e->img_cat_b.holds(p.x, p.fake)) {
      CHK(cat_cast_transpose(p.cat0, p.rows, p.K0, e->dcat_b.r() + row0 * e->dcat_b.ld, e->dcat_b.ld, p.want_w ? e->dcat_b.t() : (__bf16*)nullptr,
                             p.want_w ? e->dcat_b.ldt : 0L, s));
      e->img_cat_b.built(p.x, p.fake);
    }
  } else if (p.split) {
    const int ld = e->ld_adv2 = p.fs.ld_adv;
    CHK(e->adv2.ensure((size_t)2 * N * ld * sizeof(float)));
    float* dst = e->adv2.as<float>() + row0 * ld;
    if (both || !e->img_adv2.holds(nullptr, p.fake)) {
      BuildAdvArgs ba;
      memset(&ba, 0, sizeof(ba));
      ba.fa = p.cat0.fa; ba.fb = p.cat0.fb; ba.ldf = p.ldf; ba.idx = e->d_adv_cols; ba.na = e->Da; ba.out = dst; ba.ldo = ld; ba.split = N; ba.rows = p.rows;
      if (tv) tv->ride_on(e, ba);
      launch_build_adv(ba, s);
      LAUNCH_CHECK();
      if (tv) CHK(tv->rode(e, s));
      e->img_adv2.built(nullptr, p.fake);
    }
    p.fs.adv = dst;
    if (p.want_w) CHK(pitched_rows(e, e->dx_pitched, p.x, p.fs.ldx, p.fs.cd, N, &p.fs.xp, &p.fs.ldxp, s));
  } else if (p.needs_f32_image) {
    CHK(e->dcat.ensure((size_t)2 * N * p.ldc * sizeof(float)));
    if (both && p.cat0.cd > 0) {
      launch_build_cat2(p.x, p.cat0.cd, p.real, p.fake, p.ldf, e->d_adv_cols, e->Da, e->dcat.as<float>(), p.ldc, N, s);
      LAUNCH_CHECK();
    } else {
      if (both) CHK(build_cat(e, p.x, p.real, p.ldf, 0, N, p.ldc, s));
      if (both || !e->img_cat.holds(p.x, p.fake)) CHK(build_cat(e, p.x, p.fake, p.ldf, N, N, p.ldc, s));
    }
    e->img_cat.built(p.x, p.fake);
    p.img = e->dcat.as<float>() + row0 * p.ldc;
  }
  return GT_OK;
}

static int d_pass_forward(gt_engine* e, DPass& p, hipStream_t s) {
  CHK(sn_prepare_pass(e, s));
  switch (p.kind) {
    case D_SRU:
      CHK(sru_stack_forward(e, GT_ROLE_D, p.img, p.ldc, p.nseq, p.T, p.passes, p.npass, s, &p.top, &p.ld_top, p.sru_d16 ? &p.cat0 : nullptr, p.want_w));
      p.H = p.ld_top;
      break;
    case D_LSTM:
      CHK(lstm_check_lengths(e, p.B, p.T));
      CHK(lstm_stack_forward(e, GT_ROLE_D, p.img, p.ldc, p.nseq, p.T, p.passes, p.npass, s, &p.top, &p.ld_top));
      p.H = p.ld_top;
      break;
    case D_MLP_B16:
      CHK(refresh_shadows(e, GT_ROLE_D, false, s));
      CHK(stack_forward_b16(e, GT_ROLE_D, e->dcat_b.r() + (p.npass == 2 ? 0 : p.N) * e->dcat_b.ld, e->dcat_b.ld, p.rows, p.passes, p.npass, p.N,
                            e->ws[GT_ROLE_D].specs, p.want_w, s));
      break;
    case D_MLP_F32:
      CHK(stack_forward(e, GT_ROLE_D, p.img, p.ldc, p.rows, p.passes, p.npass, p.N, e->ws[GT_ROLE_D].specs, s, p.split ? &p.fs : nullptr, p.fused ? 1 : 1 << 30));
      break;
  }
  return GT_OK;
}

static int d_pass_head(gt_engine* e, DPass& p, const HeadCall& c_in, float* dst, hipStream_t s) {
  const int H = p.H;
  NetWs& W = e->ws[GT_ROLE_D];
  CHK(e->dzA.ensure((size_t)2 * p.N * std::max(H, 1) * sizeof(float)));
  CHK(e->dzB.ensure((size_t)2 * p.N * std::max(H, 1) * sizeof(float)));
  HeadCall c = c_in;
  c.objective = e->gan_objective;
  if (p.fused) return run_dstack(e, c, p.npass == 1 ? dst : nullptr, s);
  HeadAct a;
  memset(&a, 0, sizeof(a));
  a.K = H; a.has_act = true; a.dH = e->dzA.as<float>();
  switch (p.kind) {
    case D_SRU: case D_LSTM:
      CHK(W.dout.ensure((size_t)2 * p.rows * H * sizeof(float)));
      a.H = p.top; a.has_act = false; a.spec = no_drop(); a.dH = W.dout.as<float>();
      break;
    case D_MLP_B16:
      a.H = W.actb.back().r(); a.h_ld = W.actb.back().ld; a.spec = W.specs.back();
      if (c.want_grad) { CHK(e->dz_b[0].ensure(p.rows, H, p.want_w)); a.dz_img = &e->dz_b[0]; a.dz_t = p.want_w; }
      break;
    case D_MLP_F32:
      a.H = W.act.back().as<float>(); a.spec = W.specs.back();
      break;
  }
  return run_head(e, c, a, s);
}

static int d_pass_backward(gt_engine* e, DPass& p, float* dst, hipStream_t s) {
  if (p.fused && p.npass == 1) return GT_OK;
  const long N = p.N, row0 = p.npass == 2 ? N : 0;
  const int col0 = cond_dim(e), Da = e->Da;
  switch (p.kind) {
    case D_SRU:
      return sru_stack_backward(e, GT_ROLE_D, p.img, p.ldc, p.nseq, p.T, p.passes, p.npass, p.want_w, dst, s);
    case D_LSTM: {
      float* dx0 = nullptr;
      if (dst) { CHK(e->d_dx0.ensure((size_t)2 * N * p.K0 * sizeof(float))); dx0 = e->d_dx0.as<float>(); }
      CHK(lstm_stack_backward(e, GT_ROLE_D, p.img, p.ldc, p.nseq, p.T, p.passes, p.npass, p.want_w, dx0, s));
      if (dst) {
        launch_copy_cols(dx0 + row0 * p.K0, p.K0, col0, dst, Da, 0, N, Da, s);
        LAUNCH_CHECK();
      }
      return GT_OK;
    }
    case D_MLP_B16:
      return stack_backward_b16(e, GT_ROLE_D, p.want_w ? e->dcat_b.t() : (__bf16*)nullptr, p.want_w ? e->dcat_b.ldt : 0, p.rows, e->ws[GT_ROLE_D].specs, 0,
                                p.want_w, dst, Da, col0, Da, row0, N, s);
    case D_MLP_F32:
      return stack_backward(e, GT_ROLE_D, p.img, p.ldc, p.rows, e->ws[GT_ROLE_D].specs, e->dzA.as<float>(), e->dzB.as<float>(), p.want_w, dst, Da, col0, Da,
                            row0, N, s, p.split ? &p.fs : nullptr);
  }
  return GT_OK;
}

static int d_pass_penalty(gt_engine* e, DPass& p, const float* mask, hipStream_t s) {
  GpState& G = e->gp;
  if (G.kind == GP_OFF) return GT_OK;
  Net& D = e->net[GT_ROLE_D];
  NetWs& W = e->ws[GT_ROLE_D];
  const long N = p.N;
  const int L = (int)D.hidden.size(), H = D.d.hidden_dim, cd = cond_dim(e), Da = e->Da, ld_g = (Da + 3) & ~3;
  if (p.kind != D_MLP_F32 || L < 1 || Da < 1) return fail(GT_ERR_INVALID, "gradient penalty: float32 MLP discriminator only");
  CHK(slab_defer_flush(W.sdefer, s));
  G.stream = s;
  if (G.kind == GP_WGAN) {
    float* img = p.split ? e->adv2.as<float>() : e->dcat.as<float>();
    const int ldo = p.split ? p.fs.ld_adv : p.ldc, col0 = p.split ? 0 : cd;
    uint32_t k0, k1;
    gp_eps_keys(e, &k0, &k1);
    CHK(G.eps.ensure((size_t)N * sizeof(float)));
    CHK(launch_gp_interp(p.real, p.fake, p.ldf, e->d_adv_cols, Da, G.eps_inj, k0, k1, img, ldo, col0, N, G.eps.as<float>(), s));
    G.img = img; G.img_ld = ldo; G.img_col0 = col0; G.img_rows = N;
    const int pass3[1] = {3};
    CHK(stack_forward(e, GT_ROLE_D, p.img, p.ldc, N, pass3, 1, N, W.specs, s, p.split ? &p.fs : nullptr));
  }
  CHK(G.g.ensure((size_t)N * ld_g * sizeof(float)));
  CHK(G.dw0.ensure((size_t)H * Da * sizeof(float)));
  const int nblk = gp_row_blocks(N);
  CHK(G.part.ensure((size_t)2 * nblk * sizeof(double)));
  GpCall c;
  memset(&c, 0, sizeof(c));
  c.L = L; c.cd = cd; c.Da = Da; c.kind = G.kind; c.prec = product_prec(e, GT_ROLE_D); c.weight = G.weight; c.rows = N;
  for (int l = 0; l < L; ++l) {
    const Lin& Lr = D.hidden[l];
    if (Lr.out != H) return fail(GT_ERR_INVALID, "gradient penalty: hidden layers of one width only");
    GpLayer& q = c.l[l];
    q.W = Lr.W; q.dW = Lr.dW; q.in = Lr.in; q.out = Lr.out;
    q.H = W.act[l].as<float>(); q.spec = W.specs[l];
    q.a = W.act[l].as<float>() + N * (long)Lr.out;
    q.c = (l & 1) ? e->dzB.as<float>() : e->dzA.as<float>();
  }
  c.w_last = D.last.W; c.dw_last = D.last.dW;
  c.g = G.g.as<float>(); c.ld_g = ld_g;
  c.mask = mask; c.inv_tv_dev = LossNormaliser::inv_tv(e->sc());
  c.part = G.part.as<double>(); c.part_cap = (long)(G.part.bytes / sizeof(double));
  c.rec = G.rec.as<double>();
  c.dw0s = G.dw0.as<float>();
  c.slabs = &e->slabs; c.colp = &e->colp;
  return launch_grad_penalty(c, s);
}

int KeptLeak::claim(gt_engine* e, const float* y_hat_static, long N, float** out) {
  const Net& G = e->net[GT_ROLE_G];
  *out = nullptr;
  if (!(G.bound && G.d.grads && e->g_pass_valid && y_hat_static == e->last_yhs && e->N == N)) return GT_OK;
  if (pending) return fail(GT_ERR_STATE, "update_discriminator called twice without optimizer_g.zero_grad() (train.py:538)");
  CHK(buf.ensure((size_t)N * e->Da * sizeof(float)));
  *out = buf.as<float>();
  return GT_OK;
}

extern "C" int gt_update_discriminator_begin(gt_engine* e, const float* x, const float* y_static, const float* y_hat_static,
                                             const float* mask, int B, int T, int train, float eps, void* stream) {
  CHK(check_common(e, B, T));
  Net& D = e->net[GT_ROLE_D];
  if (!D.bound) return fail(GT_ERR_STATE, "discriminator not bound");
  if (!y_static || !y_hat_static || !mask) return fail(GT_ERR_INVALID, "null tensor");
  CHK(check_gan_objective(e));
  CHK(gp_refusals(e));
  hipStream_t s = (hipStream_t)stream;
  const long N = (long)B * T;
  const bool tr = train != 0;
  ResultsChannel& rc = e->results;
  const bool plain_early = rc.early && !comm_on(e), comm_early = rc.early && comm_on(e);
  DPass p;
  CHK(d_pass_plan(e, x, y_static, y_hat_static, e->Ds, 2, B, T, tr, &p));
  if (comm_on(e) && tr && D.grads_dirty)
    return fail(GT_ERR_STATE, "data-parallel step: optimizer_d.zero_grad() must precede update_discriminator (the gradient buckets are summed over the ranks in place)");
  if (e->sn.on && tr && D.grads_dirty)
    return fail(GT_ERR_STATE, "spectral norm: optimizer_d.zero_grad() must precede update_discriminator (the last step's gradient was projected in place)");
  e->ws[GT_ROLE_D].sdefer.reset(rc.early && tr && D.has_opt);
  const TvPlan tv(e, p, mask, tr && D.has_opt && D.d.grads);
  e->norm.d_step_begins(tv.route == TvPlan::IN_SUMS);
  CHK(tv.before_input(e, s));
  CHK(d_pass_input(e, p, &tv, s));
  CHK(d_pass_forward(e, p, s));
  if (tr && !D.d.grads) return fail(GT_ERR_STATE, "phase == \"train\" but the discriminator was bound without grads");
  HeadCall hc;
  memset(&hc, 0, sizeof(hc));
  hc.mode = HEAD_D_STEP; hc.rows = p.rows; hc.n_real = N; hc.mask = mask; hc.n_mask = N; hc.eps = eps; hc.want_grad = tr; hc.want_w = tr;
  if (plain_early) { hc.early_res = rc.target(); hc.ticket = rc.take_ticket(); }
  CHK(tv.before_head(e, hc, s));
  CHK(d_pass_head(e, p, hc, nullptr, s));
  rc.clear_early();
  if (plain_early) CHK(rc.post_early(s, hc.ticket));
  if (comm_early) CHK(comm_early_results(e, GT_ROLE_D, tv.early_sums(e->sc()), tv.n_early_sums(), 0.f, 0.f, 0.f, s));
  if (tr) {
    CHK(comm_grads_ready(e, GT_ROLE_D, D.last.dW, (long)D.last.in * D.last.out + D.last.out, s));
    float* leak;
    CHK(e->leak.claim(e, y_hat_static, N, &leak));
    CHK(d_pass_backward(e, p, leak, s));
    CHK(d_pass_penalty(e, p, mask, s));
    D.grads_dirty = true;
    if (leak) e->leak.kept(tv.route == TvPlan::IN_SUMS);
  }
  CHK(comm_finish_step(e, GT_ROLE_D, tr, &e->sc()->s_real, comm_early ? 0 : 4, s));
  rc.begin_done[GT_ROLE_D] = true;
  return GT_OK;
}

static void fill_d_result(const StepResults* h, gt_d_result* out) {
  out->loss_d = h->loss_d; out->loss_fake_d = h->loss_fake_d; out->loss_real_d = h->loss_real_d;
  out->real_correct_count = h->real_correct; out->fake_correct_count = h->fake_correct;
  out->grad_norm = h->gnorm_d;
}
static void fill_g_result(const StepResults* h, gt_g_result* out) {
  out->loss_mse = h->loss_mse; out->loss_mge = h->loss_mge; out->loss_adv = h->loss_adv;
  out->loss_g = h->loss_g; out->grad_norm = h->gnorm_g;
}

template <typename Finalize>
static int step_end(gt_engine* e, int role, bool train, bool out_is_null, hipStream_t s, Finalize finalize) {
  if (!e) return fail(GT_ERR_INVALID, "null argument");
  ResultsChannel& rc = e->results;
  if (!rc.begin_done[role]) return fail(GT_ERR_STATE, "gt_update_%s_end without _begin", role == GT_ROLE_D ? "discriminator" : "generator");
  rc.begin_done[role] = false;
  if (out_is_null && rc.early_posted()) return fail(GT_ERR_STATE, "deferred results are a split-phase feature");
  if (train) CHK(optimizer_step(e, role, role == GT_ROLE_D ? &e->sc()->gnorm2_d : &e->sc()->gnorm2_g, s));
  if (rc.early_posted()) return rc.wait_early();
  finalize();
  LAUNCH_CHECK();
  return out_is_null ? rc.post_deferred(role, s) : rc.fetch(s);
}
static int step_result(gt_engine* e, int role) { return e->results.collect(role); }

extern "C" int gt_update_discriminator_end(gt_engine* e, int train, gt_d_result* out, void* stream) {
  hipStream_t s = (hipStream_t)stream;
  CHK(step_end(e, GT_ROLE_D, train != 0, !out, s, [&] { launch_finalize_d(e->sc(), e->res(), train ? 0 : 1, 0, s); }));
  if (out) fill_d_result(e->results.h_res, out);
  return GT_OK;
}
extern "C" int gt_update_discriminator_result(gt_engine* e, gt_d_result* out) {
  if (!e || !out) return fail(GT_ERR_INVALID, "null argument");
  CHK(step_result(e, GT_ROLE_D));
  fill_d_result(e->results.h_def[GT_ROLE_D], out);
  return GT_OK;
}

extern "C" int gt_update_discriminator(gt_engine* e, const float* x, const float* y_static, const float* y_hat_static,
                                       const float* mask, int B, int T, int train, float eps, gt_d_result* out, void* stream) {
  if (!e) return fail(GT_ERR_INVALID, "null engine");
  e->results.early = true;
  int r = gt_update_discriminator_begin(e, x, y_static, y_hat_static, mask, B, T, train, eps, stream);
  e->results.early = false;
  if (r != GT_OK) { e->results.abandon(); e->norm.d_step_begins(false); return r; }
  return gt_update_discriminator_end(e, train, out, stream);
}

static int sum_sqerr(gt_engine* e, const float* a, int lda, const float* b, int ldb, const float* mask, long rows, int D,
                     double* out, float* g, int ldg, float gscale, hipStream_t s, int* deferred_blocks = nullptr) {
  CHK(e->partial.ensure(4096 * sizeof(double)));
  double* part = e->partial.as<double>() + 1024;
  SqerrArgs q;
  memset(&q, 0, sizeof(q));
  q.a = a; q.lda = lda; q.b = b; q.ldb = ldb; q.mask = mask; q.rows = rows; q.D = D; q.partial = part; q.g = g; q.ldg = ldg; q.gscale = gscale; q.sc = e->sc();
  const int nblk = launch_masked_sqerr(q, s);
  LAUNCH_CHECK();
  if (deferred_blocks) { *deferred_blocks = nblk; return GT_OK; }
  launch_sum_partials(part, nblk, out, s);
  LAUNCH_CHECK();
  return GT_OK;
}

static int generator_backward(gt_engine* e, const float* x, const float* y, const float* y_hat, const float* mask,
                              float mse_w, hipStream_t s) {
  Net& G = e->net[GT_ROLE_G];
  NetWs& W = e->ws[GT_ROLE_G];
  const long N = e->N;
  const int B = e->B, T = e->T, Do = G.d.out_dim;
  const bool mlp_body = !(has_lstm_body(G.d.arch) || G.d.arch == GT_ARCH_SRU);
  const int ldgy = mlp_body && e->g_band ? (Do + 3) & ~3 : Do;
  CHK(e->gy.ensure((size_t)N * ldgy * sizeof(float)));
  float* gy = e->gy.as<float>();
  const float* gs = e->gs.as<float>();
// ... 267 lines not shown
```

gantts_amd/csrc/engine_internal.hip.h:

```cpp
#pragma once
#include <hip/hip_runtime.h>
#include <math.h>
#include <stdarg.h>
#include <stdio.h>
#include <stdlib.h>
#include <string.h>
#include <algorithm>
#include <map>
#include <mutex>
#include <string>
#include <vector>

#pragma GCC visibility push(default)
#include "../../include/gantts_hip.h"
#pragma GCC visibility pop
#include "frame_kernels.hip.h"
#include "frame_args.hip.h"
#include "gemm_f32.hip.h"
#include "gemm_bf16s.hip.h"
#include "sru_args.hip.h"

using namespace gt;

int fail(int code, const char* fmt, ...);
#define HIPCHK(expr)                                                                         \
  do {                                                                                       \
    hipError_t _e = (expr);                                                                  \
    if (_e != hipSuccess)                                                                    \
      return fail(GT_ERR_HIP, "%s failed: %s (%s:%d)", #expr, hipGetErrorString(_e), __FILE__, __LINE__); \
  } while (0)
#define CHK(expr)            \
  do {                       \
    int _r = (expr);         \
    if (_r != GT_OK) return _r; \
  } while (0)
#define LAUNCH_CHECK() HIPCHK(hipGetLastError())

static inline bool env_flag(const char* name, bool dflt) { const char* v = getenv(name); return v && v[0] ? v[0] != '0' : dflt; }
static inline int cdiv(long a, long b) { return (int)((a + b - 1) / b); }
static inline int pad8(long n) { return (int)((n + 7) & ~7L); }

int ensure_dyn_lds(const void* kernel, size_t bytes);
int gemm_cu_count();

struct GtTuning {
  int gemm_pair = 1;
  int pair_order = 1;
  int gemm_tiles_big = 0;
  int gemm_unaligned = 1;
  int tn_wgs = 512;
  int split_fused = 1;
  int tn_split_wgs = 1024;
  int b16_tiles = 0;
  int b16_wg_tile = 0;
  int b16_dma = 1;
  int mlpg_fpl = 2;
  int head_vec = 0;
  int mlpg_tt = 0;
  int leak_rider = 1;
  int sru_cs_waves = 0;
  int sru_coop = 1;
  int lstm_bt = 0;
};
GtTuning& gt_tuning();

struct GemmProfiler {
  bool on = false;
  int only_kind = -1;
  bool wants(int kind) const { return on && (only_kind < 0 || only_kind == kind); }
  struct Rec { int kind, bn, am; double flops, bytes; hipEvent_t e0, e1; };
  double last_bytes[GT_PROFILE_SLOTS] = {};
  std::vector<Rec> recs;
  std::vector<hipEvent_t> pool;
  hipEvent_t get() {
    if (!pool.empty()) { hipEvent_t e = pool.back(); pool.pop_back(); return e; }
    hipEvent_t e; (void)hipEventCreate(&e); return e;
  }
};
extern GemmProfiler g_prof;

struct Scratch {
  void* p = nullptr;
  size_t bytes = 0;
  int ensure(size_t need) {
    if (need <= bytes) return GT_OK;
    if (p) { HIPCHK(hipDeviceSynchronize()); HIPCHK(hipFree(p)); p = nullptr; bytes = 0; }
    const size_t cap = need + need / 8;
    HIPCHK(hipMalloc(&p, cap));
    bytes = cap;
    return GT_OK;
  }
  void release() { if (p) { (void)hipFree(p); p = nullptr; bytes = 0; } }
  template <typename T> T* as() const { return (T*)p; }
};

struct SlabDefer {
  Scratch pool;
  size_t used = 0;
  SlabJobs jobs;
  int blocks = 0;
  bool active = false;
  SlabDefer() { jobs.n = 0; jobs.pad_ = 0; }
  void reset(bool on) { jobs.n = 0; blocks = 0; used = 0; active = on; }
};

struct Lin { float *W, *b, *dW, *db; int in, out; };
struct B16Img {
  Scratch rm, tr;
  int ld = 0; long ldt = 0;
  __bf16* r() { return rm.as<__bf16>(); }
  __bf16* t() { return tr.as<__bf16>(); }
  int ensure(long rows, int cols, bool want_t) {
    ld = pad8(cols); ldt = pad8(rows);
    CHK(rm.ensure((size_t)rows * ld * 2 + 64));
    if (want_t) CHK(tr.ensure((size_t)cols * ldt * 2 + 64));
    return GT_OK;
  }
  void release() { rm.release(); tr.release(); }
};
struct LinShadow {
  Scratch w, wt; int ldw = 0, ldwt = 0;
  __bf16* r() const { return w.as<__bf16>(); }
  __bf16* t() const { return wt.as<__bf16>(); }
  int ensure(int out, int in) {
    ldw = pad8(in); ldwt = pad8(out);
    CHK(w.ensure((size_t)out * ldw * 2 + 64));
    CHK(wt.ensure((size_t)in * ldwt * 2 + 64));
    return GT_OK;
  }
  void release() { w.release(); wt.release(); }
};
static inline bool is_i2o(int arch) { return arch == GT_ARCH_IN2OUT || arch == GT_ARCH_IN2OUT_RNN; }
static inline bool has_lstm_body(int arch) { return arch == GT_ARCH_LSTM || arch == GT_ARCH_IN2OUT_RNN; }
struct LstmDirP { float *Wih, *Whh, *bih, *bhh, *dWih, *dWhh, *dbih, *dbhh; };
struct LstmLayerP { int in; LstmDirP d[2]; };
struct SruLayerP { int in, k; float *W, *b, *dW, *db; };

struct OptimScalarCache { bool valid = false; long step = 0; float mu_product = 1.f; };

struct Net {
  bool bound = false;
  gt_model_desc d;
  std::vector<Lin> hidden;
  Lin last, gate;
  std::vector<LstmLayerP> lstm;
// ... 98 lines not shown
  double* h_out = nullptr;
  double* record() const { return rec.as<double>(); }
  double* dist() const { return rec.as<double>() + GT_LEDGER_SLOTS; }
  int* col_stat() const { return (int*)((char*)rec.p + off_tab); }
  int* col_role() const { return col_stat() + Ds; }
  double* partials() const { return (double*)((char*)rec.p + off_part); }
  void release() { rec.release(); len.release(); if (h_out) (void)hipHostFree(h_out); h_out = nullptr; configured = false; }
};

struct SnLayerDesc { long w_off; int out, in; };
struct SnPlan;
struct SnBufs { double *t, *r, *sp, *s; float* sigma; };
struct SnState {
  bool on = false;
  float *u = nullptr, *v = nullptr;
  SnPlan* plan = nullptr;
  Scratch weff, ws;
  SnBufs bufs = {nullptr, nullptr, nullptr, nullptr, nullptr};
};

namespace gt { enum GpKind { GP_OFF = 0, GP_R1 = 1, GP_WGAN = 2 }; }
struct GpLayer {
  const float* W; float* dW; int in, out;
  const float* H; gt::DropoutSpec spec;
  float* a; float* c;
};
struct GpCall {
  int L, cd, Da, kind, prec; float weight; long rows;
  GpLayer l[16];
  const float* w_last; float* dw_last;
  float* g; int ld_g; float* g_copy;
  const float* mask; const float* inv_tv_dev; float inv_tv;
  float* phi; float* nrm;
  double* part; long part_cap;
  double* sums; double* rec;
  float* dw0s;
  Scratch* slabs; Scratch* colp;
};
struct GpState {
  int kind = 0; float weight = 0.f;
  const float* eps_inj = nullptr;
  Scratch g, dw0, part, rec, eps;
  hipStream_t stream = nullptr;
  const float* img = nullptr; int img_ld = 0, img_col0 = 0; long img_rows = 0;
  void release() { g.release(); dw0.release(); part.release(); rec.release(); eps.release(); }
};

struct LossNormaliser {
  float override() const { return ovr; }
  const double* total_dev() const { return dev; }
  bool given() const { return dev || ovr > 0.f; }
  double* reduced() const { return total.as<double>(); }
  bool known(const float* m, long N) const { return mask == m && n == N && memo_ovr == ovr; }
  void note(const float* m, long N) { mask = m; n = N; memo_ovr = ovr; }
  void forget() { mask = nullptr; }      void overwritten() { forget(); }
  void set_override(float tv) { ovr = tv; dev = nullptr; }
  void set_total_dev(const double* p) { dev = p; forget(); }
  int attach() { return total.ensure(64); }      void release() { total.release(); }
  int start(gt_engine* e, const float* m, long N, hipStream_t s);
  int send(gt_engine* e, hipStream_t s);
  int join(gt_engine* e, hipStream_t s);
  int file(gt_engine* e, const float* m, long N, const double* from, hipStream_t s);
  int ensure(gt_engine* e, const float* m, long N, hipStream_t s);
  void d_step_begins(bool unnormalised) { d_unnorm = unnormalised; }
  bool d_unnormalised() const { return d_unnorm; }
  const float* take_d_scale(StepScalars* sc) { const bool u = d_unnorm; d_unnorm = false; return u ? &sc->inv_tv : (const float*)nullptr; }
  static const float* inv_tv(StepScalars* sc) { return &sc->inv_tv; }
 private:
  float ovr = -1.f; const double* dev = nullptr;
  const float* mask = nullptr; long n = 0; float memo_ovr = 0.f;
  Scratch total; bool d_unnorm = false;
};

struct KeptLeak {
  int claim(gt_engine* e, const float* y_hat_static, long N, float** out);
  void kept(bool unnormalised) { pending = true; unnorm = unnormalised; }
  const float* get() const { return pending ? buf.as<float>() : (const float*)nullptr; }
  bool unnormalised() const { return pending && unnorm; }
  void drop() { pending = unnorm = false; }      void release() { buf.release(); }
 private:
  Scratch buf; bool pending = false, unnorm = false;
};

struct gt_engine {
  gt_stream_config cfg;
  Net net[2];
  uint64_t seed = 0x5DEECE66DULL;
  uint64_t step_counter = 0;
  LossNormaliser norm;
  KeptLeak leak;
  int Dout_cfg = 0, Ds = 0, Da = 0;
  std::vector<int> h_scol, h_sstride, h_adv_cols, h_adv_inv;
  int *d_scol = nullptr, *d_sstride = nullptr, *d_adv_cols = nullptr, *d_adv_inv = nullptr;
  int *d_scol_i2o = nullptr, *d_sstride_i2o = nullptr; int i2o_ds = 0;
  MlpgCache mlpg;
  Scratch mlpg_var_ws;
  NetWs ws[2];
  Scratch dcat, dzA, dzB, gadv, gs, gy, slabs, colp, partial, headp, headw, dmask, tx, gx, dgx, dtz, dout;
  Scratch scal;
  ResultsChannel results;
  EpochLedger ledger;
  int B = 0, T = 0; long N = 0;
  const float* last_x = nullptr; const float* last_yhat = nullptr; const float* last_yhs = nullptr;
  bool g_pass_valid = false;
  const MlpgBand* g_band = nullptr;
  struct DImage {
    bool valid = false; const float* x = nullptr; const float* yhs = nullptr;
    bool holds(const float* x_, const float* yhs_) const { return valid && x == x_ && yhs == yhs_; }
    void built(const float* x_, const float* yhs_) { valid = true; x = x_; yhs = yhs_; }
  };
  DImage img_cat, img_cat_b, img_adv2;
  bool g_has_adv = false;
  Scratch i2o_gout, d_dx0;
  Scratch l_state, l_xch, s_du, s_dx, s_dbias;
  struct GtComm* comm = nullptr;
  struct GtIpc* ipc = nullptr;
  bool opt_comm_ipc = env_flag("GT_COMM_IPC", true);
  int dp_rank = 0, dp_world = 1;
  int chk_B = 0, chk_T = 0;
  std::vector<std::pair<long, long>> comm_done[2];
  std::vector<std::pair<long, long>> comm_pending[2];
  B16Img xin_b, dcat_b, gy_b, dz_b[2], fwd_b;
  Scratch d_pre;
  Scratch adv2; int ld_adv2 = 0;
  int opt_fused_dstack = getenv("GT_FUSED_DSTACK") ? atoi(getenv("GT_FUSED_DSTACK")) : 1;
  bool opt_split_first = env_flag("GT_D_SPLIT", true);
  bool opt_comm_d_one_msg = env_flag("GT_COMM_D_ONE_MSG", true), opt_comm_early_g = env_flag("GT_COMM_EARLY_G", true),
       opt_comm_force = getenv("GT_COMM_FORCE_COLLECTIVES") != nullptr;
  bool opt_comm_close_inline = env_flag("GT_COMM_CLOSE_INLINE", true);
  bool opt_comm_tv_in_sums = env_flag("GT_COMM_TV_IN_SUMS", true);
  bool opt_poll_results = env_flag("GT_POLL_RESULTS", true);
  bool opt_launch_riders = env_flag("GT_LAUNCH_RIDERS", true);
  int ld_gx = 0, ld_cx = 0;
  StepCopy dx_pitched, gx_pitched, cx_dense;
  Scratch gx_dense; bool gx_dense_on = false;
  unsigned int* h_fault_dev = nullptr;
  unsigned int* d_fault = nullptr;
  unsigned int* h_fault = nullptr;
  bool lstm_persistent = getenv("GT_LSTM_STEPS") == nullptr;
  int lstm_fwd_upc = 0;
  bool lstm_xcd_local = getenv("GT_LSTM_NO_XCD_LOCAL") == nullptr;
  int64_t lstm_paths[GT_LSTM_PATH_SLOTS] = {};
  bool matmul_bf16 = false;
  static constexpr int LEN_RING = 4;
  int* len_host[LEN_RING] = {nullptr, nullptr, nullptr, nullptr};
  Scratch len_dev[LEN_RING];
  hipEvent_t len_ev[LEN_RING] = {nullptr, nullptr, nullptr, nullptr};
  int len_cap = 0, len_slot = -1;
  int* d_lengths() { return len_slot < 0 ? nullptr : len_dev[len_slot].as<int>(); }
  bool sru_d_bf16 = env_flag("GT_SRU_D_BF16", false);
  int gan_objective = 0;
  float weight_clip[2] = {0.f, 0.f};
  struct ParamEma { float* buf = nullptr; long n = 0; double decay = 0.0; long count = 0; } ema;
  SnState sn;
  GpState gp;
  std::vector<int> h_lengths;
  StepScalars* sc() { return scal.as<StepScalars>(); }
  StepResults* res() { return (StepResults*)((char*)scal.p + 256); }
};
static inline void invalidate_d_images(gt_engine* e) { e->img_cat.valid = e->img_cat_b.valid = e->img_adv2.valid = false; }

int check_common(gt_engine* e, int B, int T);
int fault_seen(gt_engine* e);
int optim_check_desc(const gt_optim_desc_ex* od);
void optim_desc_copy(const gt_optim_desc_ex* in, gt_optim_desc_ex* out);
int launch_optim_step(const gt_optim_desc_ex& od, long step, bool buf_live, OptimScalarCache* cache, float* params, float* grads, long n,
                      const double* part, int n_partial, double* norm2_out, const unsigned int* fault_dev, unsigned int* fault_host,
                      unsigned int* skipped_host, const float* gscale, hipStream_t s, float weight_clip = 0.f, float* ema = nullptr,
                      float ema_w = 0.f, bool ema_first = false);
int param_ema_check_decay(const char* who, double decay);
static inline float param_ema_weight(double decay) { return (float)(1.0 - decay); }
int check_param_ema(const gt_engine* e);
int check_gan_objective(const gt_engine* e);
void optim_host_scalars(const gt_optim_desc_ex& od, long t, OptimScalarCache* cache, double out[2]);
gt::DropoutSpec philox_site_spec(gt_engine* e, int role, int pass, int layer, uint64_t step, float p, long half_rows = 0);
gt::DropoutSpec drop_spec(gt_engine* e, int role, int pass, int layer, const float* stacked_mask, int ld, long half_rows = 0);

int product_prec(const gt_engine* e, int role);
enum { GEMM_PATH_PAIR = 576, GEMM_PATH_TN_PAIR = 580, GEMM_PATH_REDUCE4 = 582, GEMM_PATH_REDUCE = 583, GEMM_PATH_REDUCE_SMALL = 584,
       GEMM_PATH_COLSUM_PARTIAL = 585, GEMM_PATH_COLSUM_FINALIZE = 586, GEMM_PATH_REDUCE_MULTI = 587 };
static_assert(GEMM_PATH_REDUCE_MULTI + 1 == GT_GEMM_PATH_SLOTS, "gt_gemm_path_counts slots");
constexpr int gemm_path_slot(int kind, int bm, int bn, bool va, bool vb, int prec, int amode) {
  return (((((kind * 2 + (bm == 128)) * 2 + (bn == 128)) * 2 + va) * 2 + vb) * 2 + (prec == gt::PREC_BF16)) * 6 + (amode + 1);
}
void gemm_path_count(int slot);
bool gemm_vec_ok(const float* p, int ld, bool k_contiguous = false);
bool gemm_wide_store_ok(int kind, const gt::GemmArgs& g);
bool gemm_small_tiles_ok();
namespace gt { struct DStackArgs; }
bool dstack_hidden_ok(int hidden_dim);
int dstack_panels(long rows);
int launch_dstack(const gt::DStackArgs& a, int hidden_dim, hipStream_t s, int objective = 0);
int launch_dstack_objective(const gt::DStackArgs& a, int hidden_dim, int objective, hipStream_t s);
enum { HEAD_PATH_F32 = 0, HEAD_PATH_VEC = 4, HEAD_PATH_IMG = 7, HEAD_PATH_DSTACK128 = 11, HEAD_PATH_DSTACK256 = 12, HEAD_PATH_FINALIZE64 = 13,
       HEAD_PATH_FINALIZE16 = 14 };
static_assert(HEAD_PATH_FINALIZE16 + 1 == GT_HEAD_PATH_SLOTS, "gt_head_path_counts slots");
void head_path_count(int slot);
namespace gt { struct HeadCall; struct HeadSums; struct HeadArgs; struct DStackCall; }
int launch_head_finalize(const gt::HeadCall& c, const gt::HeadSums& o, int nblk, int K, hipStream_t s);
int launch_d_head(const gt::HeadArgs& a, hipStream_t s);
int launch_d_head_objective(const gt::HeadArgs& a, int nblk, hipStream_t s);
int launch_dstack_pass(const gt::DStackCall& k, hipStream_t s);
gt::DropoutSpec no_drop();
int launch_gemm(int kind, const gt::GemmArgs& g, int prec, hipStream_t s);
int plain_product(int kind, const float* A, int lda, const float* B, int ldb, float* C, int ldc, long M, int N, int K, bool accumulate, int prec,
                  hipStream_t s);
int linear_forward(const float* X, int ldx, const float* W, int ldw, const float* b, float* Y, int ldy, long rows, int in, int out, int act,
                   const gt::DropoutSpec& drop, int prec, hipStream_t s, const float* addm = nullptr, int ld_addm = 0, long addm_wrap = 0,
                   bool accumulate = false);
int linear_forward_seg(const float* x, int ldx, long wrap, int cd, const float* adv, int ld_adv, long rows, const float* W, int ldw, int in,
                       const float* b, float* Y, int ldy, int out, int act, const gt::DropoutSpec& drop, int prec, hipStream_t s);
gt::GemmArgs backward_data_args(const float* dZ, int lddz, const float* W, int ldw, int col0, float* dX, int lddx,
                                long rows, int out, int ncols, int act_prev, const float* H, int ldh, const gt::DropoutSpec& drop);
int linear_backward_data(const float* dZ, int lddz, const float* W, int ldw, int col0, float* dX, int lddx,
                         long rows, int out, int ncols, int act_prev, const float* H, int ldh, const gt::DropoutSpec& drop, int prec, hipStream_t s);
struct SlabSet {
  float* base; float* bias;
  long stride; size_t bytes;
  int nslab, out;
  bool can4;
  SlabDefer* defer;
};
int slab_defer_flush(SlabDefer& d, hipStream_t s);
int slab_place(SlabDefer* defer, Scratch& slabs, int nslab, int out, int in, const float* dW, bool accumulate, hipStream_t s, SlabSet* set);
int slab_combine(const SlabSet& set, float* dW, float* db, bool accumulate, hipStream_t s);
int linear_backward_weight(const float* dZ, int lddz, const float* X, int ldx, long rows, int out, int in,
                           float* dW, float* db, bool accumulate, Scratch& slabs, Scratch& colp, int prec, hipStream_t s,
                           SlabDefer* defer = nullptr, const gt::GemmArgs* ride_along = nullptr, bool* rode = nullptr);
int linear_backward_weight_split(const float* dZ, int lddz, long rows, long wrap, const float* xp, int ldxp, int cd,
                                 const float* adv, int ld_adv, int Da, int out, float* dW, float* db, bool accumulate,
                                 Scratch& slabs, int prec, hipStream_t s, SlabDefer* defer, const GemmArgs* rider = nullptr, bool* rode = nullptr);

gt::GemmB16Args b16_args();
enum { B16_PATH_CAST_F32 = 60, B16_PATH_CAST_BF16 = 61, B16_PATH_CAST_SEQDROP = 62, B16_PATH_CAST_MULTI = 63, B16_PATH_CAST_CAT = 64,
       B16_PATH_CAST_CATDROP = 65 };
static_assert(B16_PATH_CAST_CATDROP + 1 == GT_GEMM_B16_PATH_SLOTS, "gt_gemm_b16_path_counts slots");
constexpr int b16_path_slot(int epi, int amode, int form) { return (epi * 5 + amode) * 4 + form; }
void b16_path_count(int slot);
int launch_gemm_b16(const gt::GemmB16Args& g, int nslab, hipStream_t s, int tile = 0);
int cast_transpose(const float* in, int ld_in, long rows, int cols, __bf16* out, int ldo, __bf16* outT, long ldt,
                   float* colsum, bool colsum_accumulate, Scratch* colp, hipStream_t s);
int cast_transpose(const __bf16* in, int ld_in, long rows, int cols, __bf16* out, int ldo, __bf16* outT, long ldt,
                   float* colsum, bool colsum_accumulate, Scratch* colp, hipStream_t s);
int cast_jobs_add(gt::CastJobs& jobs, int& blocks, const float* in, int ldi, long rows, int cols, __bf16* out, int ldo, __bf16* outT, long ldt);
int cast_transpose_multi(const gt::CastJobs& jobs, int blocks, hipStream_t s);
int seqdrop_cast_transpose(const gt::SeqDropSrc& src, long rows, int cols, __bf16* out, int ldo, __bf16* outT, long ldt, hipStream_t s);
int cat_cast_transpose(const gt::CatSrc& src, long rows, int cols, __bf16* out, int ldo, __bf16* outT, long ldt, hipStream_t s);
int catdrop_cast_transpose(const gt::CatDropSrc& src, long rows, int cols, __bf16* out, int ldo, __bf16* outT, long ldt, hipStream_t s);
int weight_grad_b16(const __bf16* dZT, long lddzt, const __bf16* XT, long ldxt, long rows, int out, int in, float* dW, float* db,
                    bool accumulate, Scratch& slabs, hipStream_t s, SlabDefer* defer = nullptr);
int shadow_cast(LinShadow& sh, const float* W, int r0, int out, int in, hipStream_t s);
struct B16Dst {
  float* C = nullptr; int ldc = 0; B16Img* img = nullptr; bool twin = false, accumulate = false;
  B16Dst(float* C_, int ldc_, bool accumulate_ = false) : C(C_), ldc(ldc_), accumulate(accumulate_) {}
  B16Dst(B16Img& img_, bool twin_) : img(&img_), twin(twin_) {}
};
int b16_forward(const __bf16* X, int ldx, long rows, const __bf16* W, int ldw, int n, int k, const float* bias, int act,
                const gt::DropoutSpec& drop, const B16Dst& dst, hipStream_t s);
int b16_backward_data(const __bf16* dZ, int lddz, long rows, const __bf16* W, int ldw, int n, int k, int act_prev, const B16Img* H,
                      const gt::DropoutSpec& drop, const B16Dst& dst, hipStream_t s);

int ensure_band(gt_engine* e, const float* R, int T, hipStream_t s, const MlpgBand** out);
int mlpg_forward(gt_engine* e, const float* y, int ldy, const int* scol, const int* sstride, int Ds,
                 float* ys, int ldys, int B, int T, const MlpgBand& band, hipStream_t s);
int mlpg_backward(gt_engine* e, const float* gs, int ldgs, const int* scol, const int* sstride, int Ds,
                  float* gy, int ldgy, int B, int T, float mse_w, const float* yhat, const float* ytgt, int ldt,
                  const float* mask, const MlpgBand& band, hipStream_t s);

int cond_dim(gt_engine* e);
struct OutTop { const float* x = nullptr; int ld = 0; B16Img* img = nullptr; const LinShadow* sh = nullptr; bool img_ready = false, want_t = false; };
struct OutGrad { B16Dst to; int act_prev; gt::DropoutSpec drop; bool ride; };
int out_layer_forward(gt_engine* e, int role, const OutTop& top, long rows, float* out, hipStream_t s);
int out_layer_backward(gt_engine* e, int role, const float* gy, int ldgy, long rows, const OutTop& top, const OutGrad& dst, SlabDefer* defer,
                       hipStream_t s);

int sn_plan_build(const SnLayerDesc* layers, int n, long n_flat, SnPlan** out);
void sn_plan_free(SnPlan* p);
long sn_plan_sum_out(const SnPlan* p);
long sn_plan_sum_in(const SnPlan* p);
int sn_plan_partials(const SnPlan* p);
size_t sn_plan_bytes(const SnPlan* p);
SnBufs sn_plan_bufs(const SnPlan* p, void* ws);
int launch_sn_prepare(const SnPlan* p, const float* W, float* u, float* v, float* weff, const SnBufs& b, bool iterate, hipStream_t s);
int launch_sn_project(const SnPlan* p, float* G, const float* weff, const float* u, const float* v, const SnBufs& b, double* norm_part, hipStream_t s);
void sn_point_weights(gt_engine* e);
int sn_rebind(gt_engine* e);
int sn_prepare_pass(gt_engine* e, hipStream_t s);
int sn_project_grads(gt_engine* e, double* norm_part, int* n_partial, hipStream_t s);

int gp_row_blocks(long rows);
void gp_eps_keys(const gt_engine* e, uint32_t* key0, uint32_t* key1);
int launch_gp_interp(const float* real, const float* fake, int ldf, const int* idx, int na, const float* eps_in, uint32_t key0, uint32_t key1,
                     float* out, int ldo, int col0, long rows, float* eps_out, hipStream_t s);
int launch_grad_penalty(const GpCall& c, hipStream_t s);
int gp_refusals(const gt_engine* e);

struct GtComm {
  void* comm = nullptr;
  int rank = 0, world = 1;
  hipStream_t stream = nullptr;
  hipEvent_t ev[8] = {nullptr, nullptr, nullptr, nullptr, nullptr, nullptr, nullptr, nullptr};
  int next_ev = 0;
  hipEvent_t ev_done = nullptr;
  struct TraceRec { int kind, inl; double bytes; hipEvent_t e0, e1; bool closed; };
  bool trace = false;
  long trace_dropped = 0;
  std::vector<TraceRec> trec;
};
bool comm_on(const gt_engine* e);
int comm_grads_ready(gt_engine* e, int role, const float* lo, long count, hipStream_t compute);
int comm_flush(gt_engine* e, int role, hipStream_t compute, bool closing = false);
// ... 33 lines not shown
```

gantts_amd/csrc/frame_kernels.hip.h:

```cpp
#pragma once
#include <hip/hip_runtime.h>
#include <stdint.h>
#include "gemm_f32.hip.h"
#include "gan_objective.hip.h"

namespace gt {

constexpr int RED_THREADS = 256;

__device__ __forceinline__ float wave_sum(float v) {
#pragma unroll
  for (int o = 32; o > 0; o >>= 1) v += __shfl_xor(v, o, 64);
  return v;
}
__device__ __forceinline__ double wave_sum_d(double v) {
#pragma unroll
  for (int o = 32; o > 0; o >>= 1) v += __shfl_xor(v, o, 64);
  return v;
}
__device__ __forceinline__ float block_sum(float v, float* sh) {
  v = wave_sum(v);
  const int lane = threadIdx.x & 63, w = threadIdx.x >> 6;
  __syncthreads();
  if (lane == 0) sh[w] = v;
// ... 385 lines not shown
        if (lane == 0) dbs += (double)dz;
        float vals[KP];
#pragma unroll
        for (int j = 0; j < KP; ++j) {
          const int k = kof[j];
          const float hv = hrow[ri][j];
          dwacc[j] = fmaf(dz, hv, dwacc[j]);
          float f = 1.f;
          if (has_act) {
            bool keep = ((keepb[j] >> ri) & 1u) != 0u;
            if (drop.mode == DROP_BUFFER) keep = drop.mask[(long)r * drop.ld_mask + kidx[j]] != 0.f;
            f = leaky_drop_grad(hv, keep, drop.mode == DROP_NONE ? 1.f : drop.scale);
          }
          const float val = dz * wreg[j] * f;
          vals[j] = val;
          if (B16OUT) outv[ri][j] = val;
          if (!VEC && k < K) {
            if (dH) dH[(long)r * lddh + k] = val;
            if (B16OUT && dHb) dHb[(long)r * lddhb + k] = (__bf16)val;
          }
        }
        if constexpr (VEC) {
          if (dH) {
#pragma unroll
            for (int jj = 0; jj < KP / 4; ++jj) {
              float* dst = dH + (long)r * lddh + kof[4 * jj];
              if (kof[4 * jj] + 3 < K) {
                f32x4 v;
#pragma unroll
                for (int q = 0; q < 4; ++q) v[q] = vals[4 * jj + q];
                st4u(dst, v);
              } else {
#pragma unroll
                for (int q = 0; q < 4; ++q) if (kof[4 * jj + q] < K) dst[q] = vals[4 * jj + q];
              }
            }
          }
        }
      }
    }
    if (B16OUT && want_grad && dHbT) {
#pragma unroll
      for (int j = 0; j < KP; ++j) {
        const int k = kof[j];
        if (k >= K) continue;
#pragma unroll
        for (int q = 0; q < 2; ++q) {
          const int rs = 16 * g + 8 * q + 4 * h;
          __bf16* dst = dHbT + (long)k * lddhbt + rs;
          if (rs + 3 < n_rows) {
            bf16x4 pk;
#pragma unroll
            for (int s4 = 0; s4 < 4; ++s4) pk[s4] = (__bf16)outv[B16OUT ? 4 * q + s4 : 0][j];
            *reinterpret_cast<bf16x4*>(dst) = pk;
          } else {
#pragma unroll
            for (int s4 = 0; s4 < 4; ++s4) if (rs + s4 < n_rows) dst[s4] = (__bf16)outv[B16OUT ? 4 * q + s4 : 0][j];
          }
        }
      }
    }
  }
  if (lane == 0) { shd[0][wv] = s_real; shd[1][wv] = s_fake; shd[2][wv] = n_rok; shd[3][wv] = n_fok; shd[4][wv] = dbs; }
  if (want_grad && dw_partial) {
#pragma unroll
    for (int j = 0; j < KP; ++j) { const int k = kof[j]; if (k < K) smf[wv * K + k] = dwacc[j]; }
  }
  __syncthreads();
  if (threadIdx.x == 0) {
    HeadPartials p;
    p.s_real = shd[0][0] + shd[0][1] + shd[0][2] + shd[0][3];
    p.s_fake = shd[1][0] + shd[1][1] + shd[1][2] + shd[1][3];
    p.n_real_ok = shd[2][0] + shd[2][1] + shd[2][2] + shd[2][3];
    p.n_fake_ok = shd[3][0] + shd[3][1] + shd[3][2] + shd[3][3];
    p.db = shd[4][0] + shd[4][1] + shd[4][2] + shd[4][3];
    hp[blockIdx.x] = p;
  }
  if (want_grad && dw_partial) {
    for (int k = threadIdx.x; k < K; k += blockDim.x)
      dw_partial[(long)blockIdx.x * K + k] = (smf[k] + smf[K + k]) + (smf[2 * K + k] + smf[3 * K + k]);
  }
}

static __global__ __launch_bounds__(1024) void d_head_finalize_kernel(const HeadPartials* __restrict__ hp, const float* __restrict__ dw_partial,
                                                               int nblk, int K, int mode, StepScalars* sc,
                                                               float* __restrict__ dw, float* __restrict__ db, int accumulate,
                                                               StepResults* early_res ,
                                                               unsigned* ticket = nullptr, unsigned ticket_value = 0,
                                                               int cgw = 64 ,
                                                               int scal_blk = 0 ) {
  __shared__ float shw[1024];
  __shared__ double shd[16];
  const int nparts = (int)blockDim.x / cgw;
  const int kl = threadIdx.x % cgw, part = threadIdx.x / cgw;
  const int k = blockIdx.x * cgw + kl;
  if (dw) {
    float sa[16];
#pragma unroll
    for (int u = 0; u < 16; ++u) sa[u] = 0.f;
    if (k < K) {
      int i = part;
      for (; i + 15 * nparts < nblk; i += 16 * nparts) {
#pragma unroll
        for (int u = 0; u < 16; ++u) sa[u] += dw_partial[(long)(i + nparts * u) * K + k];
      }
      for (; i < nblk; i += nparts) sa[0] += dw_partial[(long)i * K + k];
    }
#pragma unroll
    for (int u = 0; u < 8; ++u) sa[u] += sa[u + 8];
#pragma unroll
    for (int u = 0; u < 4; ++u) sa[u] += sa[u + 4];
    shw[part * cgw + kl] = (sa[0] + sa[1]) + (sa[2] + sa[3]);
    __syncthreads();
    if (part == 0 && k < K) {
      float tot = 0.f;
      for (int q = 0; q < nparts; ++q) tot += shw[q * cgw + kl];
      dw[k] = accumulate ? dw[k] + tot : tot;
    }
  }
  if ((int)blockIdx.x == scal_blk) {
    double v[5] = {0, 0, 0, 0, 0};
    for (int i = threadIdx.x; i < nblk; i += blockDim.x) {
      v[0] += hp[i].s_real; v[1] += hp[i].s_fake; v[2] += hp[i].n_real_ok; v[3] += hp[i].n_fake_ok; v[4] += hp[i].db;
    }
    double r[5];
    for (int q = 0; q < 5; ++q) r[q] = block_sum_d(v[q], shd);
    if (threadIdx.x == 0) {
      if (mode == HEAD_D_STEP) {
        sc->s_real = r[0]; sc->s_fake = r[1]; sc->n_real_ok = r[2]; sc->n_fake_ok = r[3];
        if (early_res) {
          const float T = sc->tv;
          const float lr = -((float)r[0]) / T, lf = -((float)r[1]) / T;
          early_res->loss_real_d = lr; early_res->loss_fake_d = lf; early_res->loss_d = lr + lf;
          early_res->real_correct = (float)r[2]; early_res->fake_correct = (float)r[3];
          early_res->gnorm_d = 0.f; early_res->tv = T;
          publish_ticket(ticket, ticket_value);
        }
      } else sc->s_adv = r[0];
      if (db) db[0] = accumulate ? db[0] + (float)r[4] : (float)r[4];
    }
  }
}


struct GFinalize {
  int on;
  StepScalars* sc;
  StepResults* out;
  float adv_w, mse_w, mge_w;
  int has_adv;
  const double* part_mge; int n_mge;
  const double* part_mse; int n_mse;
  const HeadPartials* hp; int n_hp;
  unsigned* ticket; unsigned ticket_value;
};
__device__ __forceinline__ void finalize_g_body(StepScalars* sc, StepResults* out, float adv_w, float mse_w, float mge_w, int has_adv,
                                                int zero_gnorm, const double* __restrict__ part_mge, int n_mge,
                                                const double* __restrict__ part_mse, int n_mse,
                                                const HeadPartials* __restrict__ hp, int n_hp, double* shp ,
                                                unsigned* ticket = nullptr, unsigned ticket_value = 0) {
  if (part_mge || part_mse || hp) {
    if (part_mge) {
      double v = 0.0;
      for (int i = threadIdx.x; i < n_mge; i += blockDim.x) v += __builtin_nontemporal_load(part_mge + i);
      const double t = block_sum_d(v, shp);
      if (threadIdx.x == 0) sc->s_mge = t;
    }
    if (part_mse) {
      double v = 0.0;
      for (int i = threadIdx.x; i < n_mse; i += blockDim.x) v += __builtin_nontemporal_load(part_mse + i);
      const double t = block_sum_d(v, shp);
      if (threadIdx.x == 0) sc->s_mse = t;
    }
    if (hp) {
      double v = 0.0;
      for (int i = threadIdx.x; i < n_hp; i += blockDim.x) v += hp[i].s_real;
      const double t = block_sum_d(v, shp);
      if (threadIdx.x == 0) sc->s_adv = t;
    }
    __syncthreads();
  }
  if (threadIdx.x || !out) return;
  const float T = sc->tv;
  const float mse = (float)sc->s_mse / T, mge = (float)sc->s_mge / T;
  const float adv = has_adv ? -((float)sc->s_adv) / T : 0.f;
  out->loss_mse = mse; out->loss_mge = mge; out->loss_adv = adv;
  out->loss_g = (mse_w * mse + mge_w * mge) + adv_w * adv;
  out->gnorm_g = zero_gnorm ? 0.f : (float)sqrt(sc->gnorm2_g); out->tv = T;
  publish_ticket(ticket, ticket_value);
}

static __global__ __launch_bounds__(RED_THREADS) void static_grad_kernel(
    const float* __restrict__ yhs, int ld1, const float* __restrict__ ys, int ld2,
    const float* __restrict__ mask, long rows, int Ds, float mge_w,
    const int* __restrict__ adv_inv , const float* __restrict__ leak, int ldl,
    const float* __restrict__ gadv, int lda, float adv_w,
    float* __restrict__ gs, int ldg, double* __restrict__ partial, StepScalars* __restrict__ sc, const GFinalize fin,
    int leak_unnorm ) {
  __shared__ double sh[16];
  int nblk = gridDim.x;
  const int blk = blockIdx.x;
  if (fin.on) {
    if (blockIdx.x == gridDim.x - 1) {
      finalize_g_body(fin.sc, fin.out, fin.adv_w, fin.mse_w, fin.mge_w, fin.has_adv, 1, fin.part_mge, fin.n_mge, fin.part_mse, fin.n_mse,
                      fin.hp, fin.n_hp, sh, fin.ticket, fin.ticket_value);
      return;
    }
    --nblk;
  }
  double acc = 0.0;
  const long total = rows * Ds;
  const float sc2 = 2.f * mge_w * sc->inv_tv;
  const float leak_s = leak_unnorm ? sc->inv_tv : 1.f;
  const long stride = (long)nblk * blockDim.x;
  const long sr = stride / Ds;
  const int sd = (int)(stride - sr * Ds);
  long e = (long)blk * blockDim.x + threadIdx.x;
  long r = e / Ds;
  int c = (int)(e - r * Ds);
  for (; e + 3 * stride < total; e += 4 * stride) {
    long rr[4];
    int cc[4];
#pragma unroll
    for (int u = 0; u < 4; ++u) {
      if (c >= Ds) { c -= Ds; ++r; }
// ... 370 lines not shown
```

gantts_amd/csrc/gemm_f32.hip.h:

```cpp
#pragma once
#include <hip/hip_runtime.h>
#include <stdint.h>
#include <type_traits>

namespace gt {

typedef float f32x16 __attribute__((ext_vector_type(16)));
typedef float f32x4 __attribute__((ext_vector_type(4)));
typedef __bf16 bf16x8 __attribute__((ext_vector_type(8)));
typedef __bf16 bf16x4 __attribute__((ext_vector_type(4)));

struct __attribute__((packed, aligned(4))) F4U { float v[4]; };
__device__ __forceinline__ f32x4 ld4u(const float* p) {
  const F4U t = *reinterpret_cast<const F4U*>(p);
  f32x4 r; r[0] = t.v[0]; r[1] = t.v[1]; r[2] = t.v[2]; r[3] = t.v[3];
  return r;
}
__device__ __forceinline__ void st4u(float* p, const f32x4& r) {
  F4U t; t.v[0] = r[0]; t.v[1] = r[1]; t.v[2] = r[2]; t.v[3] = r[3];
  *reinterpret_cast<F4U*>(p) = t;
}

enum GemmPrec { PREC_F32 = 0, PREC_BF16 = 1 };
constexpr int GEMM_KP = 40;
// ... 640 lines not shown
  for (; kt + 2 < nk; ++kt) k_tile(kt, T_{}, F_{});
  if (kt + 2 == nk) {
    if (has_tail) k_tile(kt, T_{}, T_{}); else k_tile(kt, T_{}, F_{});
    ++kt;
  }
  if (kt + 1 == nk) k_tile(kt, F_{}, F_{});
  }
  };
  gemm_kloop_prio(true);
  prologue();
  k_loop();
  gemm_kloop_prio(false);

  if (KIND == GEMM_TN && want_csum) {
    constexpr int OWN = BM / VWA;
#pragma unroll
    for (int c = 0; c < VWA; ++c) smem[tid * VWA + c] = csum[c];
    __syncthreads();
    if (tid < BM && m0 + tid < g.M) {
      const int own = tid / VWA, c = tid % VWA;
      float tot = 0.f;
#pragma unroll
      for (int j = 0; j < GEMM_THREADS / OWN; ++j) tot += smem[(own + j * OWN) * VWA + c];
      g.colsum_slab[(long)slab * g.M + m0 + tid] = tot;
    }
  }

#ifdef GT_ABLATE_NO_EPILOGUE
  {
    float v = 0.f;
#pragma unroll
    for (int i = 0; i < TM; ++i)
#pragma unroll
      for (int j = 0; j < TN_; ++j)
#pragma unroll
        for (int r = 0; r < 16; ++r) v += acc[i][j][r];
    g.C[(long)(m0 + wm * WM + l31) * g.ldc + n0 + wn * WN + half] = v;
    return;
  }
#endif
  if constexpr (KIND == GEMM_NT && AMODE == GEMM_A_LEAKY_PHILOX_SEG) {
    const int nh = g.dual_rows > 0 ? 2 : 1;
    f32x16 acc0[TM][TN_];
    if (nh > 1) {
#pragma unroll
      for (int i = 0; i < TM; ++i)
#pragma unroll
        for (int j = 0; j < TN_; ++j) acc0[i][j] = acc[i][j];
    }
    for (int h = 0; h < nh; ++h) {
      if (h > 0) {
        __syncthreads();
#pragma unroll
        for (int i = 0; i < TM; ++i)
#pragma unroll
          for (int j = 0; j < TN_; ++j) acc[i][j] = acc0[i][j];
      }
#pragma unroll
      for (int u = 0; u < UA; ++u) {
        int kk, mm; a_pos(u, kk, mm);
        offA[u] = (uint32_t)min(m0 + mm, mclamp) * (uint32_t)g.lda_seg + (uint32_t)kk;
      }
      pA = g.A_seg + (long)h * g.dual_rows * g.lda_seg;
      pB = g.B_seg;
      k_begin = 0; k_end = g.K_seg;
      nk = (k_end + GEMM_BK - 1) / GEMM_BK;
      has_tail = (k_end % GEMM_BK) != 0;
      gemm_kloop_prio(true);
      prologue();
      k_loop();
      gemm_kloop_prio(false);
      gemm_store_tile<KIND, BM, BN, PREC, AMODE>(g, slab, m0 + h * g.dual_rows, n0, acc, smem, nh > 1 ? (h + 1) * g.dual_rows : g.M);
    }
    return;
  }
  gemm_store_tile<KIND, BM, BN, PREC, AMODE>(g, slab, m0, n0, acc, smem, g.M);
}

__device__ __forceinline__ int gemm_xcd_order(int bid, int nwg) {
  const int q = nwg >> 3, r = nwg & 7, xcd = bid & 7, idx = bid >> 3;
  return (xcd < r ? xcd * (q + 1) : r * (q + 1) + (xcd - r) * q) + idx;
}

template <int PREC, int AMODE = GEMM_A_RUNTIME>
__global__ __launch_bounds__(GEMM_THREADS, 4) void gemm_pair_kernel(const GemmArgs g1, const GemmArgs g2, const int n1, const int tn_first) {
  extern __shared__ __attribute__((aligned(16))) float smem[];
  int bid = blockIdx.x;
  const int n2 = (int)gridDim.x - n1;
  const bool is_nn = tn_first ? bid >= n2 : bid < n1;
  if (is_nn) {
    bid = gemm_xcd_order(tn_first ? bid - n2 : bid, n1);
    const int tile_m = bid / g1.n_tiles_n, tile_n = bid - tile_m * g1.n_tiles_n;
    gemm_tile<GEMM_NN, 64, 64, true, true, PREC, AMODE>(g1, 0, tile_m, tile_n, smem);
  } else {
    bid = gemm_xcd_order(tn_first ? bid : bid - n1, n2);
    const int tiles_mn = g2.n_tiles_m * g2.n_tiles_n;
    const int slab = bid / tiles_mn, t = bid - slab * tiles_mn;
    const int tile_m = t / g2.n_tiles_n, tile_n = t - tile_m * g2.n_tiles_n;
    gemm_tile<GEMM_TN, 64, 64, true, true, PREC>(g2, slab, tile_m, tile_n, smem);
  }
}

template <int PREC>
__global__ __launch_bounds__(GEMM_THREADS, 4) void gemm_tn_pair_kernel(const GemmArgs g1, const GemmArgs g2, const int n1, const GemmArgs g3, const int n3) {
  extern __shared__ __attribute__((aligned(16))) float smem[];
  int bid = blockIdx.x;
  if (bid >= (int)gridDim.x - n3) {
    bid -= (int)gridDim.x - n3;
    gemm_tile<GEMM_NN, 64, 64, true, false, PREC, GEMM_A_NONE>(g3, 0, bid / g3.n_tiles_n, bid % g3.n_tiles_n, smem);
    return;
  }
  const int n2 = (int)gridDim.x - n3 - n1;
  if (bid >= n2) {
    bid = gemm_xcd_order(bid - n2, n1);
    const int tiles_mn = g1.n_tiles_m * g1.n_tiles_n;
    const int slab = bid / tiles_mn, t = bid - slab * tiles_mn;
    gemm_tile<GEMM_TN, 64, 64, true, true, PREC, GEMM_A_TN_SUM2>(g1, slab, t / g1.n_tiles_n, t % g1.n_tiles_n, smem);
  } else {
    bid = gemm_xcd_order(bid, n2);
    const int tiles_mn = g2.n_tiles_m * g2.n_tiles_n;
    const int slab = bid / tiles_mn, t = bid - slab * tiles_mn;
    gemm_tile<GEMM_TN, 64, 64, true, true, PREC>(g2, slab, t / g2.n_tiles_n, t % g2.n_tiles_n, smem);
  }
}

#ifndef GT_SEG_WGS
#define GT_SEG_WGS 4
#endif
template <int BM, int BN, int AMODE> constexpr int gemm_min_wgs() { return (BM == 64 && BN == 64 && AMODE == GEMM_A_LEAKY_PHILOX_SEG) ? GT_SEG_WGS : 2; }
template <int KIND, int BM, int BN, bool VA, bool VB, int PREC = PREC_F32, int AMODE = GEMM_A_RUNTIME>
__global__ __launch_bounds__(GEMM_THREADS, (gemm_min_wgs<BM, BN, AMODE>())) void gemm_f32_kernel(const GemmArgs g) {
  extern __shared__ __attribute__((aligned(16))) float smem[];
  const int bid = gemm_xcd_order(blockIdx.x, gridDim.x);
  const int tiles_mn = g.n_tiles_m * g.n_tiles_n;
  const int slab = bid / tiles_mn;
  const int t = bid - slab * tiles_mn;
  const int tile_m = t / g.n_tiles_n, tile_n = t - tile_m * g.n_tiles_n;
  gemm_tile<KIND, BM, BN, VA, VB, PREC, AMODE>(g, slab, tile_m, tile_n, smem);
}

}
```

include/gantts_hip.h:

```cpp
#ifndef GANTTS_HIP_H_
#define GANTTS_HIP_H_

#include <stdint.h>

#ifdef __cplusplus
extern "C" {
#endif

#define GT_OK 0
#define GT_ERR_INVALID 1
#define GT_ERR_HIP 2
#define GT_ERR_STATE 3
#define GT_ERR_DIM 4

#define GT_ROLE_G 0
#define GT_ROLE_D 1

#define GT_ARCH_MLP 0
#define GT_ARCH_IN2OUT 1
#define GT_ARCH_LSTM 2
#define GT_ARCH_SRU 3
#define GT_ARCH_IN2OUT_RNN 4

#define GT_OPT_ADAGRAD 0
// ... 296 lines not shown
  const float* bias;
  const float* dy;
  const float* h;
  const float* mask;
  float* c;
  uint16_t* cb;
  uint16_t* cbt;
  float* dw;
  float* db;
} gt_gemm_b16_case;
int gt_op_gemm_b16(const gt_gemm_b16_case* c, void* stream);

#define GT_CAST_PLAIN_F32 0
#define GT_CAST_PLAIN_BF16 1
#define GT_CAST_SEQDROP 2
#define GT_CAST_CAT 3
#define GT_CAST_CATDROP 4
#define GT_CAST_MULTI 5
#define GT_CAST_MAX_JOBS 8
typedef struct gt_cast_job {
  const float* in;
  uint16_t* out;
  uint16_t* outT;
  int64_t rows, ldt;
  int32_t ldi, cols, ldo, pad_;
} gt_cast_job;
typedef struct gt_cast_case {
  int32_t kind, cols, ldi, ldo;
  int32_t colsum_accumulate, T, cd, ldf;
  int32_t n_jobs, pad_;
  int64_t rows, ldt, N, row_off;
  const void* in;
  uint16_t* out;
  uint16_t* outT;
  float* colsum;
  const float* mul;
  const float* x;
  const float* fa;
  const float* fb;
  const int32_t* idx;
  gt_cast_job jobs[GT_CAST_MAX_JOBS];
} gt_cast_case;
int gt_op_cast_image(const gt_cast_case* c, void* stream);

#define GT_SRU_PATH_SLOTS 13
int gt_sru_path_counts(int64_t* counts, int reset);

typedef struct gt_sru_scan_case {
  int32_t backward;
  int32_t B, T, H, dirs, k, act;
  int32_t mask_mode;
  float keep_scale, p;
  uint32_t key0, key1;
  int32_t seq_mul, seq_add;
  int32_t ldu, ldx, lddx, ld_up_add, ld_nxb, ld_dub;
  int64_t ld_nxbt, ld_dubt;
  const float* U;
  const float* x;
  const float* bias;
  float* h;
  float* c;
  const float* dh;
  float* dU;
  float* dx;
  float* dbias_part;
  const float* mask;
  const float* up_mul;
  const float* up_add;
  const float* nx_mul;
  uint16_t* nx_b;
  uint16_t* nx_bt;
  uint16_t* dU_b;
  uint16_t* dU_bt;
} gt_sru_scan_case;
int gt_op_sru_scan(const gt_sru_scan_case* c, void* stream);
int gt_op_sru_dx_adv_finish(float* dx_adv, int64_t rows, int Da, int T, const float* mul, int ld_mul, const float* hw, int ld_hw,
                            void* stream);
int gt_op_sru_input_mask(float* mul, int B, int n, float p, uint32_t key0, uint32_t key1, const float* inj, int seq_mul, int seq_add,
                         void* stream);
int gt_op_sru_input_dropout(const float* x, int ldx, float* y, int ldy, int B, int T, int n, const float* mul, void* stream);

#define GT_HEAD_PATH_SLOTS 15
int gt_head_path_counts(int64_t* counts, int reset);

#define GT_SN_MAX_LAYERS 17
#define GT_SN_PATH_SLOTS 5
typedef struct gt_sn_case {
  int32_t n_layers, iterate;
  int64_t n_flat, norm_cap;
  int64_t w_off[GT_SN_MAX_LAYERS];
  int32_t out[GT_SN_MAX_LAYERS], in[GT_SN_MAX_LAYERS];
  const float* W;
  float* u;
  float* v;
  float* weff;
  float* sigma;
  float* G;
  double* s;
  double* norm_partials;
  int32_t* n_norm_partials;
} gt_sn_case;
int gt_op_spectral_norm(const gt_sn_case* c, void* stream);
int gt_op_sn_project(const gt_sn_case* c, void* stream);
int gt_sn_path_counts(int64_t* counts, int reset);

typedef struct gt_drop_site {
  int32_t mode;
  float p;
  uint32_t key0, key1;
  uint32_t dp_t16, dp_nl16, dp_half, dp_add, dp_mul;
  float dp_inv_t16;
  int32_t ld_mask, pad_;
  const float* mask;
} gt_drop_site;

#define GT_GP_MAX_LAYERS 16
#define GT_GP_PATH_SLOTS 8
typedef struct gt_gp_case {
  int32_t kind, L, H, cd, Da, ld_g;
  int64_t rows;
  float weight, inv_tv;
  const float* W[GT_GP_MAX_LAYERS];
  float* dW[GT_GP_MAX_LAYERS];
  const float* Hact[GT_GP_MAX_LAYERS];
  float* a[GT_GP_MAX_LAYERS];
  float* c[GT_GP_MAX_LAYERS];
  gt_drop_site drop[GT_GP_MAX_LAYERS];
  const float* w_last;
  float* dw_last;
  const float* mask;
  float* g;
  float* g_copy;
  float* phi;
  float* nrm;
  double* sums;
  double* rec;
} gt_gp_case;
int gt_op_grad_penalty(const gt_gp_case* c, void* stream);
int gt_gp_path_counts(int64_t* counts, int reset);

typedef struct gt_d_head_case {
  int32_t mode, K, ldh, h_ld;
  int32_t has_act, want_grad, want_w, defer_scalars;
  int32_t accumulate, unit_tv, has_tv, lddh;
  int32_t lddhb, objective;
  float eps, tv;
  int64_t rows, n_real, n_mask, lddhbt;
  gt_drop_site drop;
  const void* H;
  const float* w;
  const float* bias;
  const float* mask;
  const double* tv_dev;
  float* Dout;
  float* dH;
  uint16_t* dHb;
  uint16_t* dHbT;
  float* dW;
  float* db;
  double* scalars;
} gt_d_head_case;
int gt_op_d_head(const gt_d_head_case* c, void* stream);

typedef struct gt_dstack_case {
  int32_t mode, L, hidden_dim, want_grad;
  int32_t accumulate, unit_tv, has_tv, ldw0;
// ... 163 lines not shown
```

Before: 12.85 million frames/s.

## Ride the D-head finalize kernel inside the last-layer backward GEMM pair launch

The discriminator head's finalize reduction (dW/db/score sums and early results) is no longer launched as its own kernel. It is parked and carried as extra workgroups in the next gemm_pair launch (backward data plus weight grad of the last D hidden layer), which saves one kernel launch and its serialization gap on the D step. The rider runs in the GEMM's 256-thread workgroups with a body unrolled 4x to cover 1024 logical threads. It adds a templated rider path and a fallback that launches the parked kernel if it was never absorbed.

```diff
diff --git a/gantts_amd/_lib.py b/gantts_amd/_lib.py
--- a/gantts_amd/_lib.py
+++ b/gantts_amd/_lib.py
@@ -23,6 +23,7 @@
 GEMM_B16_PATH_SLOTS = 66
 SRU_PATH_SLOTS = 13
 HEAD_PATH_SLOTS = 15
+RIDER_PATH_SLOTS = 2
 SN_MAX_LAYERS, SN_PATH_SLOTS = 17, 5
 GP_MAX_LAYERS, GP_PATH_SLOTS = 16, 8
 GRAD_PENALTIES = {None: 0, "r1": 1, "wgan-gp": 2}
@@ -286,6 +287,7 @@
     "gt_op_sru_input_mask": (_I, [_P, _I, _I, _F, C.c_uint32, C.c_uint32, _P, _I, _I, _P]),
     "gt_op_sru_input_dropout": (_I, [_P, _I, _P, _I, _I, _I, _I, _P, _P]),
     "gt_head_path_counts": (_I, [C.POINTER(_L), _I]),
+    "gt_rider_path_counts": (_I, [C.POINTER(_L), _I]),
     "gt_op_d_head": (_I, [C.POINTER(DHeadCase), _P]),
     "gt_op_dstack": (_I, [C.POINTER(DStackCase), _P]),
     "gt_op_frame": (_I, [C.POINTER(FrameCase), _P]),
diff --git a/gantts_amd/csrc/d_tail_args.hip.h b/gantts_amd/csrc/d_tail_args.hip.h
--- a/gantts_amd/csrc/d_tail_args.hip.h
+++ b/gantts_amd/csrc/d_tail_args.hip.h
@@ -1,5 +1,7 @@
 #pragma once
 #include "dstack_f32.hip.h"
+
+struct HeadFinalizePark;
 
 namespace gt {
 
@@ -16,6 +18,7 @@
   unsigned ticket;
   bool unit_tv;
   int objective;
+  ::HeadFinalizePark* park;
 };
 
 struct HeadSums {
diff --git a/gantts_amd/csrc/eng_core.hip b/gantts_amd/csrc/eng_core.hip
--- a/gantts_amd/csrc/eng_core.hip
+++ b/gantts_amd/csrc/eng_core.hip
@@ -431,7 +431,7 @@
     v.gemm_unaligned = geti("GT_GEMM_UNALIGNED", v.gemm_unaligned); v.tn_wgs = geti("GT_TN_WGS", v.tn_wgs); v.tn_split_wgs = geti("GT_TN_SPLIT_WGS", v.tn_split_wgs); v.split_fused = geti("GT_SPLIT_FUSED", v.split_fused);
     v.b16_tiles = geti("GT_B16_TILES", v.b16_tiles); v.b16_wg_tile = geti("GT_B16_WG_TILE", v.b16_wg_tile); v.b16_dma = geti("GT_B16_DMA", v.b16_dma);
     v.mlpg_fpl = geti("GT_MLPG_FPL", v.mlpg_fpl); v.mlpg_tt = geti("GT_MLPG_TT", v.mlpg_tt); v.sru_coop = geti("GT_SRU_COOP", v.sru_coop); v.sru_cs_waves = geti("GT_SRU_CS_WAVES", v.sru_cs_waves); v.leak_rider = geti("GT_LEAK_RIDER", v.leak_rider);
-    v.head_vec = geti("GT_HEAD_VEC", v.head_vec);
+    v.head_vec = geti("GT_HEAD_VEC", v.head_vec); v.head_rider = geti("GT_HEAD_RIDER", v.head_rider);
     v.lstm_bt = geti("GT_LSTM_BT", v.lstm_bt);
     if (v.lstm_bt != 8 && v.lstm_bt != 16) v.lstm_bt = 0;
     return v;
@@ -444,7 +444,8 @@
   struct { const char* n; int* p; } tab[] = {
       {"gemm_pair", &t.gemm_pair}, {"pair_order", &t.pair_order}, {"gemm_tiles_big", &t.gemm_tiles_big}, {"gemm_unaligned", &t.gemm_unaligned},
       {"tn_wgs", &t.tn_wgs}, {"tn_split_wgs", &t.tn_split_wgs}, {"split_fused", &t.split_fused}, {"b16_tiles", &t.b16_tiles},
-      {"b16_wg_tile", &t.b16_wg_tile}, {"b16_dma", &t.b16_dma}, {"mlpg_fpl", &t.mlpg_fpl}, {"mlpg_tt", &t.mlpg_tt}, {"sru_coop", &t.sru_coop}, {"sru_cs_waves", &t.sru_cs_waves}, {"leak_rider", &t.leak_rider}, {"head_vec", &t.head_vec}};
+      {"b16_wg_tile", &t.b16_wg_tile}, {"b16_dma", &t.b16_dma}, {"mlpg_fpl", &t.mlpg_fpl}, {"mlpg_tt", &t.mlpg_tt}, {"sru_coop", &t.sru_coop}, {"sru_cs_waves", &t.sru_cs_waves}, {"leak_rider", &t.leak_rider}, {"head_vec", &t.head_vec},
+      {"head_rider", &t.head_rider}};
   if (!strcmp(name, "lstm_bt")) {
     if (value != 0 && value != 8 && value != 16) return fail(GT_ERR_INVALID, "lstm_bt must be 0 (by shape), 8 or 16, not %d", value);
     t.lstm_bt = value;
diff --git a/gantts_amd/csrc/eng_gemm_f32.hip b/gantts_amd/csrc/eng_gemm_f32.hip
--- a/gantts_amd/csrc/eng_gemm_f32.hip
+++ b/gantts_amd/csrc/eng_gemm_f32.hip
@@ -5,7 +5,7 @@
 int launch_gemm_nt(const GemmArgs& g, int bm, int bn, int prec, hipStream_t s);
 int launch_gemm_nn(const GemmArgs& g, int bm, int bn, int prec, hipStream_t s);
 int launch_gemm_tn(const GemmArgs& g, int bm, int bn, int nslab, int prec, hipStream_t s);
-int launch_gemm_pair(const GemmArgs& nn_in, const GemmArgs& tn_in, int nslab, int prec, hipStream_t s);
+int launch_gemm_pair(const GemmArgs& nn_in, const GemmArgs& tn_in, int nslab, int prec, hipStream_t s, HeadFinalizePark* park);
 int launch_gemm_tn_pair(const GemmArgs& g1_in, const GemmArgs& g2_in, int nslab1, int nslab2, int prec, hipStream_t s, const GemmArgs* rider, bool* rode);
 int gemm_cu_count() {
   static std::map<int, int> cus;
@@ -118,6 +118,10 @@
   return gemm_pair_enabled() && gemm_small_tiles_ok() && nn.M > 64 && gemm_vec_ok(nn.A, nn.lda, true) && gemm_vec_ok(nn.B, nn.ldb);
 }
 
+
+bool linear_backward_pairs(const float* dZ, int lddz, const float* X, int ldx, const float* dW, const GemmArgs& nn) {
+  return dW && gemm_vec_ok(dZ, lddz) && gemm_vec_ok(X, ldx) && gemm_small_tiles_ok() && gemm_pair_ok(nn);
+}
 
 int slab_defer_flush(SlabDefer& d, hipStream_t s) {
   if (d.jobs.n > 0) {
@@ -178,7 +182,7 @@
 }
 int linear_backward_weight(const float* dZ, int lddz, const float* X, int ldx, long rows, int out, int in,
                                   float* dW, float* db, bool accumulate, Scratch& slabs, Scratch& colp, int prec, hipStream_t s,
-                                  SlabDefer* defer, const GemmArgs* ride_along, bool* rode) {
+                                  SlabDefer* defer, const GemmArgs* ride_along, bool* rode, HeadFinalizePark* park) {
   if (rode) *rode = false;
   if (dW) {
     const bool t64 = gemm_vec_ok(dZ, lddz) && gemm_vec_ok(X, ldx) && gemm_small_tiles_ok();
@@ -197,7 +201,7 @@
     g.k_chunk = k_chunk; g.slab_stride = set.stride;
     g.colsum_slab = db ? set.bias : nullptr;
     if (t64 && ride_along && rode && gemm_pair_ok(*ride_along)) {
-      CHK(launch_gemm_pair(*ride_along, g, nslab, prec, s));
+      CHK(launch_gemm_pair(*ride_along, g, nslab, prec, s, park));
       *rode = true;
     } else {
       CHK(launch_gemm_slabs(g, t64 ? 64 : 128, nslab, prec, s));
diff --git a/gantts_amd/csrc/eng_gemm_f32_pair.hip b/gantts_amd/csrc/eng_gemm_f32_pair.hip
--- a/gantts_amd/csrc/eng_gemm_f32_pair.hip
+++ b/gantts_amd/csrc/eng_gemm_f32_pair.hip
@@ -1,6 +1,6 @@
 #include "gemm_f32_launch.hip.h"
 
-int launch_gemm_pair(const GemmArgs& nn_in, const GemmArgs& tn_in, int nslab, int prec, hipStream_t s) {
+int launch_gemm_pair(const GemmArgs& nn_in, const GemmArgs& tn_in, int nslab, int prec, hipStream_t s, HeadFinalizePark* park) {
   GemmArgs nn = nn_in, tn = tn_in;
   nn.wide_store = gemm_wide_store_ok(GEMM_NN, nn) ? 1 : 0;
   tn.wide_store = 0;
@@ -24,10 +24,23 @@
   const int tn_first = gt_tuning().pair_order;
   const int grid = n1 + n2;
   gemm_path_count(GEMM_PATH_PAIR + (bf16 ? 3 : am == GEMM_A_NONE ? 0 : am == GEMM_A_LEAKY_PHILOX ? 1 : 2));
-  if (bf16) hipLaunchKernelGGL(gemm_pair_kernel<PREC_BF16>, dim3(grid), dim3(GEMM_THREADS), lds, s, nn, tn, n1, tn_first);
-  else if (am == GEMM_A_NONE) hipLaunchKernelGGL((gemm_pair_kernel<PREC_F32, GEMM_A_NONE>), dim3(grid), dim3(GEMM_THREADS), lds, s, nn, tn, n1, tn_first);
-  else if (am == GEMM_A_LEAKY_PHILOX) hipLaunchKernelGGL((gemm_pair_kernel<PREC_F32, GEMM_A_LEAKY_PHILOX>), dim3(grid), dim3(GEMM_THREADS), lds, s, nn, tn, n1, tn_first);
-  else      hipLaunchKernelGGL(gemm_pair_kernel<PREC_F32>, dim3(grid), dim3(GEMM_THREADS), lds, s, nn, tn, n1, tn_first);
+  static_assert(HEAD_FINALIZE_LDS <= gemm_lds_bytes<GEMM_NN, 64, 64>(), "the riding finalisation works in the pair launch's LDS");
+  if (park && park->pending && park->r.n > 0 && !bf16 && am != GEMM_A_NONE) {
+    const HeadFinalizeRider r = park->r;
+    if (am == GEMM_A_LEAKY_PHILOX) {
+      CHK(ensure_dyn_lds((const void*)gemm_pair_kernel<PREC_F32, GEMM_A_LEAKY_PHILOX, HeadFinalizeRider>, lds));
+      hipLaunchKernelGGL((gemm_pair_kernel<PREC_F32, GEMM_A_LEAKY_PHILOX, HeadFinalizeRider>), dim3(grid + r.n), dim3(GEMM_THREADS), lds, s, nn, tn, n1, tn_first, r);
+    } else {
+      CHK(ensure_dyn_lds((const void*)gemm_pair_kernel<PREC_F32, GEMM_A_RUNTIME, HeadFinalizeRider>, lds));
+      hipLaunchKernelGGL((gemm_pair_kernel<PREC_F32, GEMM_A_RUNTIME, HeadFinalizeRider>), dim3(grid + r.n), dim3(GEMM_THREADS), lds, s, nn, tn, n1, tn_first, r);
+    }
+    park->pending = false;
+    rider_path_count(RIDER_PATH_HEAD_RODE);
+  } else
+  if (bf16) hipLaunchKernelGGL(gemm_pair_kernel<PREC_BF16>, dim3(grid), dim3(GEMM_THREADS), lds, s, nn, tn, n1, tn_first, GemmNoRider{0});
+  else if (am == GEMM_A_NONE) hipLaunchKernelGGL((gemm_pair_kernel<PREC_F32, GEMM_A_NONE>), dim3(grid), dim3(GEMM_THREADS), lds, s, nn, tn, n1, tn_first, GemmNoRider{0});
+  else if (am == GEMM_A_LEAKY_PHILOX) hipLaunchKernelGGL((gemm_pair_kernel<PREC_F32, GEMM_A_LEAKY_PHILOX>), dim3(grid), dim3(GEMM_THREADS), lds, s, nn, tn, n1, tn_first, GemmNoRider{0});
+  else      hipLaunchKernelGGL(gemm_pair_kernel<PREC_F32>, dim3(grid), dim3(GEMM_THREADS), lds, s, nn, tn, n1, tn_first, GemmNoRider{0});
   LAUNCH_CHECK();
   if (g_prof.wants(5)) { HIPCHK(hipEventRecord(rec.e1, s)); g_prof.recs.push_back(rec); }
   return GT_OK;
diff --git a/gantts_amd/csrc/eng_step.hip b/gantts_amd/csrc/eng_step.hip
--- a/gantts_amd/csrc/eng_step.hip
+++ b/gantts_amd/csrc/eng_step.hip
@@ -99,7 +99,8 @@
 
 
 static int stack_backward(gt_engine* e, int role, const float* in, int ld_in, long rows, const std::vector<DropoutSpec>& specs, float* cur, float* other, bool want_w,
-                          float* dX, int lddx, int col0, int ncols, long row0, long nrows, hipStream_t s, const FirstSplit* fs = nullptr) {
+                          float* dX, int lddx, int col0, int ncols, long row0, long nrows, hipStream_t s, const FirstSplit* fs = nullptr,
+                          HeadFinalizePark* park = nullptr ) {
   Net& n = e->net[role];
   std::vector<Scratch>& acts = e->ws[role].act;
   const int L = (int)n.hidden.size(), prec = product_prec(e, role);
@@ -119,7 +120,7 @@
       CHK(comm_grads_ready(e, role, Lr.dW, (long)Lr.out * Lr.in + Lr.out, s));
     } else if (want_w) {
       CHK(linear_backward_weight(cur, Lr.out, Xin, ldx, rows, Lr.out, Lr.in, Lr.dW, Lr.db, n.grads_dirty, e->slabs, e->colp, prec, s, &e->ws[role].sdefer,
-                                 l > 0 ? &nn : nullptr, &rode));
+                                 l > 0 ? &nn : nullptr, &rode, l == L - 1 ? park : nullptr));
       CHK(comm_grads_ready(e, role, Lr.dW, (long)Lr.out * Lr.in + Lr.out, s));
       if (l == 1 && (role == GT_ROLE_G || !e->opt_comm_d_one_msg)) CHK(comm_flush(e, role, s));
     }
@@ -390,6 +391,15 @@
   }
   return GT_OK;
 }
+static std::atomic<int64_t> g_rider_paths[GT_RIDER_PATH_SLOTS];
+void rider_path_count(int slot) { g_rider_paths[slot].fetch_add(1, std::memory_order_relaxed); }
+extern "C" int gt_rider_path_counts(int64_t* counts, int reset) {
+  for (int i = 0; i < GT_RIDER_PATH_SLOTS; ++i) {
+    const int64_t v = reset ? g_rider_paths[i].exchange(0, std::memory_order_relaxed) : g_rider_paths[i].load(std::memory_order_relaxed);
+    if (counts) counts[i] = v;
+  }
+  return GT_OK;
+}
 
 int launch_head_finalize(const HeadCall& c, const HeadSums& o, int nblk, int K, hipStream_t s) {
   const bool w = c.want_grad && c.want_w;
@@ -397,11 +407,27 @@
   if (nblk > o.hp_cap || (w && (long)nblk * K > o.dw_cap)) return fail(GT_ERR_INVALID, "discriminator head: partial buffers too small for %d workgroups", nblk);
   const int cgw = (w && nblk >= 512) ? 16 : 64;
   const int n_dw = cdiv(K, cgw), extra = cgw == 16 ? 1 : 0;
-  hipLaunchKernelGGL(d_head_finalize_kernel, dim3(n_dw + extra), dim3(1024), 0, s, o.hp, o.dw_partial, nblk, K, c.mode, o.sc,
-                     w ? o.dW : (float*)nullptr, w ? o.db : (float*)nullptr, o.accumulate, c.early_res,
-                     c.ticket ? o.ticket_dev : (unsigned*)nullptr, c.ticket, cgw, extra ? n_dw : 0);
+  HeadFinalizeArgs a;
+  memset(&a, 0, sizeof(a));
+  a.hp = o.hp; a.dw_partial = o.dw_partial; a.nblk = nblk; a.K = K; a.mode = c.mode; a.sc = o.sc;
+  a.dw = w ? o.dW : (float*)nullptr; a.db = w ? o.db : (float*)nullptr; a.accumulate = o.accumulate; a.early_res = c.early_res;
+  a.ticket = c.ticket ? o.ticket_dev : (unsigned*)nullptr; a.ticket_value = c.ticket; a.cgw = cgw; a.scal_blk = extra ? n_dw : 0;
+  head_path_count(cgw == 16 ? HEAD_PATH_FINALIZE16 : HEAD_PATH_FINALIZE64);
+  if (c.park) {
+    c.park->r.a = a; c.park->r.n = n_dw + extra; c.park->pending = true;
+    return GT_OK;
+  }
+  hipLaunchKernelGGL(d_head_finalize_kernel, dim3(n_dw + extra), dim3(1024), 0, s, a);
   LAUNCH_CHECK();
-  head_path_count(cgw == 16 ? HEAD_PATH_FINALIZE16 : HEAD_PATH_FINALIZE64);
+  rider_path_count(RIDER_PATH_HEAD_OWN);
+  return GT_OK;
+}
+int head_finalize_unpark(HeadFinalizePark& park, hipStream_t s) {
+  if (!park.pending) return GT_OK;
+  park.pending = false;
+  hipLaunchKernelGGL(d_head_finalize_kernel, dim3(park.r.n), dim3(1024), 0, s, park.r.a);
+  LAUNCH_CHECK();
+  rider_path_count(RIDER_PATH_HEAD_OWN);
   return GT_OK;
 }
 
@@ -709,6 +735,22 @@
   }
   double* early_sums(StepScalars* sc) const { return route == IN_SUMS ? &sc->tv_sum : &sc->s_real; }      int n_early_sums() const { return route == IN_SUMS ? 5 : 4; }
 };
+struct HeadRide {
+  bool ride;
+  HeadRide(gt_engine* e, const DPass& p, const HeadCall& hc) {
+    const Net& D = e->net[GT_ROLE_D];
+    const int L = (int)D.hidden.size();
+    ride = p.kind == D_MLP_F32 && p.npass == 2 && p.want_w && hc.want_grad && hc.early_res && hc.ticket && e->opt_launch_riders && gt_tuning().head_rider &&
+           !comm_on(e) && !e->sn.on && e->gp.kind == GP_OFF && product_prec(e, GT_ROLE_D) == PREC_F32 && L >= 2 && e->dzA.p && e->dzB.p;
+    if (ride) {
+      const Lin& Lr = D.hidden[L - 1];
+      const float* Xin = e->ws[GT_ROLE_D].act[L - 2].as<float>();
+      const GemmArgs nn = backward_data_args(e->dzA.as<float>(), Lr.out, Lr.W, Lr.in, 0, e->dzB.as<float>(), Lr.in, p.rows, Lr.out, Lr.in, ACT_LEAKY_DROPOUT, Xin, Lr.in,
+                                             e->ws[GT_ROLE_D].specs[L - 2]);
+      ride = linear_backward_pairs(e->dzA.as<float>(), Lr.out, Xin, D.hidden[L - 2].out, Lr.dW, nn);
+    }
+  }
+};
 static int d_pass_input(gt_engine* e, DPass& p, const TvPlan* tv , hipStream_t s) {
   const long N = p.N;
   const bool both = p.npass == 2;
@@ -807,7 +849,7 @@
   return run_head(e, c, a, s);
 }
 
-static int d_pass_backward(gt_engine* e, DPass& p, float* dst, hipStream_t s) {
+static int d_pass_backward(gt_engine* e, DPass& p, float* dst, hipStream_t s, HeadFinalizePark* park = nullptr ) {
   if (p.fused && p.npass == 1) return GT_OK;
   const long N = p.N, row0 = p.npass == 2 ? N : 0;
   const int col0 = cond_dim(e), Da = e->Da;
@@ -829,7 +871,7 @@
                                 p.want_w, dst, Da, col0, Da, row0, N, s);
     case D_MLP_F32:
       return stack_backward(e, GT_ROLE_D, p.img, p.ldc, p.rows, e->ws[GT_ROLE_D].specs, e->dzA.as<float>(), e->dzB.as<float>(), p.want_w, dst, Da, col0, Da,
-                            row0, N, s, p.split ? &p.fs : nullptr);
+                            row0, N, s, p.split ? &p.fs : nullptr, park);
   }
   return GT_OK;
 }
@@ -922,6 +964,11 @@
   hc.mode = HEAD_D_STEP; hc.rows = p.rows; hc.n_real = N; hc.mask = mask; hc.n_mask = N; hc.eps = eps; hc.want_grad = tr; hc.want_w = tr;
   if (plain_early) { hc.early_res = rc.target(); hc.ticket = rc.take_ticket(); }
   CHK(tv.before_head(e, hc, s));
+  CHK(e->dzA.ensure((size_t)2 * p.N * std::max(p.H, 1) * sizeof(float)));
+  CHK(e->dzB.ensure((size_t)2 * p.N * std::max(p.H, 1) * sizeof(float)));
+  e->head_park.pending = false;
+  const HeadRide hr(e, p, hc);
+  if (hr.ride) hc.park = &e->head_park;
   CHK(d_pass_head(e, p, hc, nullptr, s));
   rc.clear_early();
   if (plain_early) CHK(rc.post_early(s, hc.ticket));
@@ -930,7 +977,8 @@
     CHK(comm_grads_ready(e, GT_ROLE_D, D.last.dW, (long)D.last.in * D.last.out + D.last.out, s));
     float* leak;
     CHK(e->leak.claim(e, y_hat_static, N, &leak));
-    CHK(d_pass_backward(e, p, leak, s));
+    CHK(d_pass_backward(e, p, leak, s, hr.ride ? &e->head_park : nullptr));
+    CHK(head_finalize_unpark(e->head_park, s));
     CHK(d_pass_penalty(e, p, mask, s));
     D.grads_dirty = true;
     if (leak) e->leak.kept(tv.route == TvPlan::IN_SUMS);
diff --git a/gantts_amd/csrc/engine_internal.hip.h b/gantts_amd/csrc/engine_internal.hip.h
--- a/gantts_amd/csrc/engine_internal.hip.h
+++ b/gantts_amd/csrc/engine_internal.hip.h
@@ -61,6 +61,7 @@
   int sru_cs_waves = 0;
   int sru_coop = 1;
   int lstm_bt = 0;
+  int head_rider = 1;
 };
 GtTuning& gt_tuning();
 
@@ -325,6 +326,11 @@
   Scratch buf; bool pending = false, unnorm = false;
 };
 
+struct HeadFinalizePark {
+  gt::HeadFinalizeRider r;
+  bool pending = false;
+};
+
 struct gt_engine {
   gt_stream_config cfg;
   Net net[2];
@@ -332,6 +338,7 @@
   uint64_t step_counter = 0;
   LossNormaliser norm;
   KeptLeak leak;
+  HeadFinalizePark head_park;
   int Dout_cfg = 0, Ds = 0, Da = 0;
   std::vector<int> h_scol, h_sstride, h_adv_cols, h_adv_inv;
   int *d_scol = nullptr, *d_sstride = nullptr, *d_adv_cols = nullptr, *d_adv_inv = nullptr;
@@ -439,6 +446,10 @@
        HEAD_PATH_FINALIZE16 = 14 };
 static_assert(HEAD_PATH_FINALIZE16 + 1 == GT_HEAD_PATH_SLOTS, "gt_head_path_counts slots");
 void head_path_count(int slot);
+enum { RIDER_PATH_HEAD_RODE = 0, RIDER_PATH_HEAD_OWN = 1 };
+static_assert(RIDER_PATH_HEAD_OWN + 1 == GT_RIDER_PATH_SLOTS, "gt_rider_path_counts slots");
+void rider_path_count(int slot);
+int head_finalize_unpark(HeadFinalizePark& park, hipStream_t s);
 namespace gt { struct HeadCall; struct HeadSums; struct HeadArgs; struct DStackCall; }
 int launch_head_finalize(const gt::HeadCall& c, const gt::HeadSums& o, int nblk, int K, hipStream_t s);
 int launch_d_head(const gt::HeadArgs& a, hipStream_t s);
@@ -469,7 +480,9 @@
 int slab_combine(const SlabSet& set, float* dW, float* db, bool accumulate, hipStream_t s);
 int linear_backward_weight(const float* dZ, int lddz, const float* X, int ldx, long rows, int out, int in,
                            float* dW, float* db, bool accumulate, Scratch& slabs, Scratch& colp, int prec, hipStream_t s,
-                           SlabDefer* defer = nullptr, const gt::GemmArgs* ride_along = nullptr, bool* rode = nullptr);
+                           SlabDefer* defer = nullptr, const gt::GemmArgs* ride_along = nullptr, bool* rode = nullptr,
+                           HeadFinalizePark* park = nullptr );
+bool linear_backward_pairs(const float* dZ, int lddz, const float* X, int ldx, const float* dW, const gt::GemmArgs& nn);
 int linear_backward_weight_split(const float* dZ, int lddz, long rows, long wrap, const float* xp, int ldxp, int cd,
                                  const float* adv, int ld_adv, int Da, int out, float* dW, float* db, bool accumulate,
                                  Scratch& slabs, int prec, hipStream_t s, SlabDefer* defer, const GemmArgs* rider = nullptr, bool* rode = nullptr);
diff --git a/gantts_amd/csrc/frame_kernels.hip.h b/gantts_amd/csrc/frame_kernels.hip.h
--- a/gantts_amd/csrc/frame_kernels.hip.h
+++ b/gantts_amd/csrc/frame_kernels.hip.h
@@ -491,65 +491,103 @@
   }
 }
 
-static __global__ __launch_bounds__(1024) void d_head_finalize_kernel(const HeadPartials* __restrict__ hp, const float* __restrict__ dw_partial,
-                                                               int nblk, int K, int mode, StepScalars* sc,
-                                                               float* __restrict__ dw, float* __restrict__ db, int accumulate,
-                                                               StepResults* early_res ,
-                                                               unsigned* ticket = nullptr, unsigned ticket_value = 0,
-                                                               int cgw = 64 ,
-                                                               int scal_blk = 0 ) {
+struct HeadFinalizeArgs {
+  const HeadPartials* hp; const float* dw_partial;
+  int nblk, K, mode;
+  StepScalars* sc;
+  float* dw; float* db; int accumulate;
+  StepResults* early_res;
+  unsigned* ticket; unsigned ticket_value;
+  int cgw;
+  int scal_blk;
+};
+template <int R>
+__device__ __forceinline__ void head_finalize_body(const HeadFinalizeArgs& a, int blk, float* shw , double* shd ) {
+  constexpr int NT = 1024, BD = NT / R;
+  const int cgw = a.cgw, nparts = NT / cgw, nblk = a.nblk, K = a.K;
+  const int kl = threadIdx.x % cgw;
+  const int k = blk * cgw + kl;
+  if (a.dw) {
+#pragma unroll
+    for (int j = 0; j < R; ++j) {
+      const int part = ((int)threadIdx.x + j * BD) / cgw;
+      float sa[16];
+#pragma unroll
+      for (int u = 0; u < 16; ++u) sa[u] = 0.f;
+      if (k < K) {
+        int i = part;
+        for (; i + 15 * nparts < nblk; i += 16 * nparts) {
+#pragma unroll
+          for (int u = 0; u < 16; ++u) sa[u] += a.dw_partial[(long)(i + nparts * u) * K + k];
+        }
+        for (; i < nblk; i += nparts) sa[0] += a.dw_partial[(long)i * K + k];
+      }
+#pragma unroll
+      for (int u = 0; u < 8; ++u) sa[u] += sa[u + 8];
+#pragma unroll
+      for (int u = 0; u < 4; ++u) sa[u] += sa[u + 4];
+      shw[part * cgw + kl] = (sa[0] + sa[1]) + (sa[2] + sa[3]);
+    }
+    __syncthreads();
+    if ((int)threadIdx.x < cgw && k < K) {
+      float tot = 0.f;
+      for (int q = 0; q < nparts; ++q) tot += shw[q * cgw + kl];
+      a.dw[k] = a.accumulate ? a.dw[k] + tot : tot;
+    }
+  }
+  if (blk == a.scal_blk) {
+    double v[R][5];
+#pragma unroll
+    for (int j = 0; j < R; ++j) {
+      for (int q = 0; q < 5; ++q) v[j][q] = 0.0;
+      for (int i = (int)threadIdx.x + j * BD; i < nblk; i += NT) {
+        v[j][0] += a.hp[i].s_real; v[j][1] += a.hp[i].s_fake; v[j][2] += a.hp[i].n_real_ok; v[j][3] += a.hp[i].n_fake_ok; v[j][4] += a.hp[i].db;
+      }
+    }
+    const int lane = threadIdx.x & 63, w = threadIdx.x >> 6;
+    double r[5];
+#pragma unroll
+    for (int q = 0; q < 5; ++q) {
+      double ws[R];
+#pragma unroll
+      for (int j = 0; j < R; ++j) ws[j] = wave_sum_d(v[j][q]);
+      __syncthreads();
+      if (lane == 0) {
+#pragma unroll
+        for (int j = 0; j < R; ++j) shd[j * (BD / 64) + w] = ws[j];
+      }
+      __syncthreads();
+      r[q] = 0.0;
+      if (threadIdx.x == 0) for (int i = 0; i < NT / 64; ++i) r[q] += shd[i];
+    }
+    if (threadIdx.x == 0) {
+      StepScalars* sc = a.sc;
+      if (a.mode == HEAD_D_STEP) {
+        sc->s_real = r[0]; sc->s_fake = r[1]; sc->n_real_ok = r[2]; sc->n_fake_ok = r[3];
+        if (a.early_res) {
+          const float T = sc->tv;
+          const float lr = -((float)r[0]) / T, lf = -((float)r[1]) / T;
+          a.early_res->loss_real_d = lr; a.early_res->loss_fake_d = lf; a.early_res->loss_d = lr + lf;
+          a.early_res->real_correct = (float)r[2]; a.early_res->fake_correct = (float)r[3];
+          a.early_res->gnorm_d = 0.f; a.early_res->tv = T;
+          publish_ticket(a.ticket, a.ticket_value);
+        }
+      } else sc->s_adv = r[0];
+      if (a.db) a.db[0] = a.accumulate ? a.db[0] + (float)r[4] : (float)r[4];
+    }
+  }
+}
+static __global__ __launch_bounds__(1024) void d_head_finalize_kernel(const HeadFinalizeArgs a) {
   __shared__ float shw[1024];
   __shared__ double shd[16];
-  const int nparts = (int)blockDim.x / cgw;
-  const int kl = threadIdx.x % cgw, part = threadIdx.x / cgw;
-  const int k = blockIdx.x * cgw + kl;
-  if (dw) {
-    float sa[16];
-#pragma unroll
-    for (int u = 0; u < 16; ++u) sa[u] = 0.f;
-    if (k < K) {
-      int i = part;
-      for (; i + 15 * nparts < nblk; i += 16 * nparts) {
-#pragma unroll
-        for (int u = 0; u < 16; ++u) sa[u] += dw_partial[(long)(i + nparts * u) * K + k];
-      }
-      for (; i < nblk; i += nparts) sa[0] += dw_partial[(long)i * K + k];
-    }
-#pragma unroll
-    for (int u = 0; u < 8; ++u) sa[u] += sa[u + 8];
-#pragma unroll
-    for (int u = 0; u < 4; ++u) sa[u] += sa[u + 4];
-    shw[part * cgw + kl] = (sa[0] + sa[1]) + (sa[2] + sa[3]);
-    __syncthreads();
-    if (part == 0 && k < K) {
-      float tot = 0.f;
-      for (int q = 0; q < nparts; ++q) tot += shw[q * cgw + kl];
-      dw[k] = accumulate ? dw[k] + tot : tot;
-    }
-  }
-  if ((int)blockIdx.x == scal_blk) {
-    double v[5] = {0, 0, 0, 0, 0};
-    for (int i = threadIdx.x; i < nblk; i += blockDim.x) {
-      v[0] += hp[i].s_real; v[1] += hp[i].s_fake; v[2] += hp[i].n_real_ok; v[3] += hp[i].n_fake_ok; v[4] += hp[i].db;
-    }
-    double r[5];
-    for (int q = 0; q < 5; ++q) r[q] = block_sum_d(v[q], shd);
-    if (threadIdx.x == 0) {
-      if (mode == HEAD_D_STEP) {
-        sc->s_real = r[0]; sc->s_fake = r[1]; sc->n_real_ok = r[2]; sc->n_fake_ok = r[3];
-        if (early_res) {
-          const float T = sc->tv;
-          const float lr = -((float)r[0]) / T, lf = -((float)r[1]) / T;
-          early_res->loss_real_d = lr; early_res->loss_fake_d = lf; early_res->loss_d = lr + lf;
-          early_res->real_correct = (float)r[2]; early_res->fake_correct = (float)r[3];
-          early_res->gnorm_d = 0.f; early_res->tv = T;
-          publish_ticket(ticket, ticket_value);
-        }
-      } else sc->s_adv = r[0];
-      if (db) db[0] = accumulate ? db[0] + (float)r[4] : (float)r[4];
-    }
-  }
-}
+  head_finalize_body<1>(a, blockIdx.x, shw, shd);
+}
+constexpr int HEAD_FINALIZE_LDS = 1024 * 4 + 16 * 8;
+struct HeadFinalizeRider {
+  HeadFinalizeArgs a;
+  int n;
+  __device__ __forceinline__ void run(int blk, float* smem) const { head_finalize_body<4>(a, blk, smem, reinterpret_cast<double*>(smem + 1024)); }
+};
 
 
 struct GFinalize {
diff --git a/gantts_amd/csrc/gemm_f32.hip.h b/gantts_amd/csrc/gemm_f32.hip.h
--- a/gantts_amd/csrc/gemm_f32.hip.h
+++ b/gantts_amd/csrc/gemm_f32.hip.h
@@ -746,11 +746,16 @@
   return (xcd < r ? xcd * (q + 1) : r * (q + 1) + (xcd - r) * q) + idx;
 }
 
-template <int PREC, int AMODE = GEMM_A_RUNTIME>
-__global__ __launch_bounds__(GEMM_THREADS, 4) void gemm_pair_kernel(const GemmArgs g1, const GemmArgs g2, const int n1, const int tn_first) {
+struct GemmNoRider { int n; };
+template <int PREC, int AMODE = GEMM_A_RUNTIME, class RIDER = GemmNoRider>
+__global__ __launch_bounds__(GEMM_THREADS, 4) void gemm_pair_kernel(const GemmArgs g1, const GemmArgs g2, const int n1, const int tn_first, const RIDER rider) {
   extern __shared__ __attribute__((aligned(16))) float smem[];
   int bid = blockIdx.x;
-  const int n2 = (int)gridDim.x - n1;
+  int n2 = (int)gridDim.x - n1;
+  if constexpr (!std::is_same<RIDER, GemmNoRider>::value) {
+    if (bid < rider.n) { rider.run(bid, smem); return; }
+    bid -= rider.n; n2 -= rider.n;
+  }
   const bool is_nn = tn_first ? bid >= n2 : bid < n1;
   if (is_nn) {
     bid = gemm_xcd_order(tn_first ? bid - n2 : bid, n1);
diff --git a/include/gantts_hip.h b/include/gantts_hip.h
--- a/include/gantts_hip.h
+++ b/include/gantts_hip.h
@@ -402,6 +402,8 @@
 
 #define GT_HEAD_PATH_SLOTS 15
 int gt_head_path_counts(int64_t* counts, int reset);
+#define GT_RIDER_PATH_SLOTS 2
+int gt_rider_path_counts(int64_t* counts, int reset);
 
 #define GT_SN_MAX_LAYERS 17
 #define GT_SN_PATH_SLOTS 5
```

After: 12.94 million frames/s, median of 6. About the same (+0.7%).
